# pkusys/Auncel

Hardware: AMD Instinct MI355X
Metric: queries/sec @ recall@10>=0.95, SIFT-10M d=128 IVF4096, 1/2/4/8 GPU (higher is better)
Workload: dtype u8

## Files before the change

### auncel_amd/capi.py

```python
import ctypes as C
import os

import numpy as np

from . import build as _build

METRIC_IP, METRIC_L2 = 0, 1
SUBSET_ID_RANGE, SUBSET_ID_MOD, SUBSET_SLICE, SUBSET_ID_BITS, SUBSET_ID_BATCH = 0, 1, 2, 5, 6
SELECTOR_AND, SELECTOR_OR, SELECTOR_ANDNOT, SELECTOR_NOT = 0, 1, 2, 3

_f32p = C.POINTER(C.c_float)
_i64p = C.POINTER(C.c_int64)
_u64p = C.POINTER(C.c_uint64)
_szp = C.POINTER(C.c_size_t)
_LIB = None

SYMBOLS = [
    "amd_ivf_last_error", "amd_ivf_device_count", "amd_ivf_create", "amd_ivf_clone", "amd_ivf_destroy", "amd_ivf_set_centroids",
    "amd_ivf_set_lists", "amd_ivf_add", "amd_ivf_ntotal", "amd_ivf_list_size", "amd_ivf_get_list", "amd_ivf_coarse",
    "amd_ivf_search_preassigned", "amd_ivf_search", "amd_ivf_scan_codes", "amd_ivf_scan_codes_at", "amd_ivf_scan_codes_range",
    "amd_ivf_scan_codes_range_results", "amd_ivf_distance_to_code", "amd_ivf_stats",
    "amd_ivf_set_queries", "amd_ivf_search_resident", "amd_ivf_search_resident_preassigned", "amd_ivf_coarse_resident", "amd_ivf_set_interdis", "amd_ivf_get_interdis",
    "amd_ivf_set_tuner", "amd_ivf_search_adaptive", "amd_ivf_search_adaptive_x", "amd_ivf_search_adaptive_pre", "amd_ivf_search_timed", "amd_ivf_search_timed_x",
    "amd_ivf_train_samples",
    "amd_ivf_train_samples_x", "amd_ivf_train_samples_pre", "amd_ivf_trace_sb", "amd_ivf_arcos_table", "amd_ivf_merge_tables",
    "amd_ivf_last_timing", "amd_ivf_last_timing_detail", "amd_ivf_last_scan_min_bytes", "amd_ivf_coarse_tie_rows", "amd_ivf_last_tie_fixed", "amd_ivf_last_filter", "amd_ivf_last_direct_out", "amd_ivf_last_coarse_pick", "amd_ivf_set_async_depth", "amd_ivf_submit_adaptive", "amd_ivf_submit_search_resident", "amd_ivf_submit_coarse_resident",
    "amd_ivf_submit_search_resident_preassigned", "amd_ivf_wait", "amd_ivf_async_counts", "amd_ivf_last_tie_redone", "amd_ivf_last_tie_patched", "amd_ivf_self_check", "amd_ivf_last_round_hints", "amd_ivf_set_byte_codes", "amd_ivf_set_option", "amd_ivf_get_option",
    "amd_ivf_kmeans",
    "amd_ivf_range_search_preassigned", "amd_ivf_range_search", "amd_ivf_range_results",
    "amd_ivf_scan_arith",
    "amd_ivf_update_lists", "amd_ivf_remove_ids", "amd_ivf_last_update", "amd_ivf_layout_digest",
    "amd_ivf_subset", "amd_ivf_last_subset",
    "amd_ivf_selector_create", "amd_ivf_selector_destroy", "amd_ivf_selector_info",
    "amd_ivf_search_selected", "amd_ivf_search_preassigned_selected", "amd_ivf_search_resident_selected",
    "amd_ivf_selector_combine", "amd_ivf_range_search_selected", "amd_ivf_range_search_preassigned_selected",
    "amd_ivf_submit_search_resident_selected",
    "amd_ivf_search_selected_each", "amd_ivf_search_preassigned_selected_each", "amd_ivf_search_resident_selected_each",
    "amd_ivf_search_exact", "amd_ivf_search_exact_resident", "amd_ivf_last_exact", "amd_ivf_last_exact_detail",
    "amd_ivf_search_exact_selected", "amd_ivf_search_exact_resident_selected",
    "amd_ivf_range_search_exact", "amd_ivf_range_search_exact_resident", "amd_ivf_range_search_exact_selected", "amd_ivf_last_range_exact",
    "amd_ivf_read_fvecs", "amd_ivf_read_ivecs", "amd_ivf_read_fbin", "amd_ivf_read_ibin", "amd_ivf_free",
]


class EngineError(RuntimeError):
    def __init__(self, code, msg):
        super().__init__(f"auncel_amd error {code}: {msg}")
        self.code = code


def _share_torch_hip_runtime():
    import importlib.util
    import sys
    if "torch" in sys.modules or os.environ.get("AUNCEL_AMD_OWN_HIP_RUNTIME"):
        return
    try:
        spec = importlib.util.find_spec("torch")
    except (ImportError, ValueError):
        return
    if spec is None or not spec.origin:
        return
    d = os.path.join(os.path.dirname(spec.origin), "lib")
    names = ("libhsa-runtime64.so", "libamdhip64.so")
    if not all(os.path.exists(os.path.join(d, n)) for n in names):
        return
    for name in names:
        try:
            _SHARED[name] = C.CDLL(os.path.join(d, name), mode=C.RTLD_GLOBAL)
        except OSError as e:
            raise ImportError(f"auncel_amd: torch's bundled {name} could not be loaded next to {sorted(_SHARED)} ({e}); set "
                              "AUNCEL_AMD_OWN_HIP_RUNTIME=1 to run the engine on ROCm's own runtime (and do not use torch's GPU "
                              "side in the same process)") from e
    if os.environ.get("AUNCEL_AMD_VERBOSE"):
        print(f"[auncel_amd] running on torch's bundled HIP runtime ({d}); AUNCEL_AMD_OWN_HIP_RUNTIME=1 keeps ROCm's", file=sys.stderr)


_SHARED = {}


def hip_runtime():
    import sys
    lib()
    if "libamdhip64.so" in _SHARED:
        return _SHARED["libamdhip64.so"]
    if "torch" in sys.modules:
        p = os.path.join(os.path.dirname(sys.modules["torch"].__file__), "lib", "libamdhip64.so")
        if os.path.exists(p):
            return C.CDLL(p)
    return C.CDLL("libamdhip64.so")


def lib():
    global _LIB
    if _LIB is None:
        if not os.path.exists(_build.LIB):
            raise ImportError(f"{_build.LIB} is missing: run `python -c 'import __graft_entry__ as g; g.build()'` "
                              "(hipcc --offload-arch=gfx950).  auncel_amd has no CPU fallback.")
        _share_torch_hip_runtime()
        L = C.CDLL(os.environ.get("AUNCEL_AMD_LIB", _build.LIB))
        L.amd_ivf_last_error.restype = C.c_char_p
        for s in SYMBOLS[1:]:
            getattr(L, s).restype = C.c_int
        L.amd_ivf_free.restype = None
        _LIB = L
    return _LIB


def _chk(rc):
    if rc != 0:
        raise EngineError(rc, lib().amd_ivf_last_error().decode())
# ... 699 lines not shown
        I = np.empty((n, k), np.int64)
        used = np.zeros(n, np.uint64)
        _chk(lib().amd_ivf_search_timed_x(self._h, C.c_size_t(n), _f(x), C.c_size_t(id_offset), C.c_size_t(k), C.c_size_t(nprobe), _f(b),
                                          coarse_mode, used.ctypes.data_as(_u64p), _f(D), _i(I)))
        return D, I, used

    def train_samples(self, start, n, max_topk, gt_D, train_num, raw, coarse_mode=0):
        gt = f32(gt_D)
        D = np.empty((n, max_topk), np.float32)
        I = np.empty((n, max_topk), np.int64)
        ptrs = (_f32p * len(raw))(*[_f(r) for r in raw])
        _chk(lib().amd_ivf_train_samples(self._h, C.c_size_t(start), C.c_size_t(n), C.c_size_t(max_topk), _f(gt),
                                         C.c_size_t(train_num), coarse_mode, ptrs, _f(D), _i(I)))
        return D, I

    def train_samples_x(self, x, id_offset, max_topk, gt_D, train_num, raw, coarse_mode=0):
        x, gt = f32(x), f32(gt_D)
        n = x.shape[0]
        D = np.empty((n, max_topk), np.float32)
        I = np.empty((n, max_topk), np.int64)
        ptrs = (_f32p * len(raw))(*[_f(r) for r in raw])
        _chk(lib().amd_ivf_train_samples_x(self._h, C.c_size_t(n), _f(x), C.c_size_t(id_offset), C.c_size_t(max_topk), _f(gt),
                                           C.c_size_t(train_num), coarse_mode, ptrs, _f(D), _i(I)))
        return D, I

    def scan_arith(self):
        return int(lib().amd_ivf_scan_arith(self._h))

    def last_timing(self):
        t = (C.c_double * 8)()
        lib().amd_ivf_last_timing(self._h, t)
        mb = C.c_double(0)
        lib().amd_ivf_last_scan_min_bytes(self._h, C.byref(mb))
        return dict(coarse_ms=t[0], scan_ms=t[1], select_ms=t[2], total_ms=t[3], scan_launches=t[4], scan_bytes=t[5],
                    slot_efficiency=t[6], rounds=t[7], scan_min_bytes=mb.value)

    PHASES = ("coarse", "scan_dense", "select_dense", "scan_thr", "select_thr", "tie_fix", "plan")

    def last_timing_detail(self):
        t = (C.c_double * 16)()
        lib().amd_ivf_last_timing_detail(self._h, t)
        d = {p: (t[2 * i], t[2 * i + 1]) for i, p in enumerate(self.PHASES)}
        d["min_bytes_dense"], d["min_bytes_thr"] = t[14], t[15]
        return d

    def coarse_tie_rows(self):
        v = C.c_uint64(0)
        _chk(lib().amd_ivf_coarse_tie_rows(self._h, C.byref(v)))
        return int(v.value)

    def coarse_resident(self, start, n, nprobe, mode=0, want_dis=True):
        keys = np.empty((n, nprobe), np.int64)
        dis = np.empty((n, nprobe), np.float32) if want_dis else None
        _chk(lib().amd_ivf_coarse_resident(self._h, C.c_size_t(start), C.c_size_t(n), C.c_size_t(nprobe), _f(dis), _i(keys), mode))
        return dis, keys

    def search_resident_preassigned(self, start, n, k, keys, out=None):
        keys = i64(keys)
        assert keys.shape[0] == n
        if out is not None:
            D, I = out
        else:
            D = np.empty((n, k), np.float32)
            I = np.empty((n, k), np.int64)
        _chk(lib().amd_ivf_search_resident_preassigned(self._h, C.c_size_t(start), C.c_size_t(n), C.c_size_t(k), C.c_size_t(keys.shape[1]),
                                                       _i(keys), _f(D), _i(I)))
        return D, I

    def last_round_hints(self):
        v = (C.c_uint64 * 2)()
        _chk(lib().amd_ivf_last_round_hints(self._h, v))
        return int(v[0]), int(v[1])

    def last_tie_redone(self):
        v = C.c_uint64(0)
        _chk(lib().amd_ivf_last_tie_redone(self._h, C.byref(v)))
        return int(v.value)

    def last_tie_patched(self):
        v = C.c_uint64(0)
        _chk(lib().amd_ivf_last_tie_patched(self._h, C.byref(v)))
        return int(v.value)

    def last_tie_fixed(self):
        v = C.c_uint64(0)
        _chk(lib().amd_ivf_last_tie_fixed(self._h, C.byref(v)))
        return int(v.value)

    def last_filter(self):
        v = (C.c_uint64 * 2)()
        _chk(lib().amd_ivf_last_filter(self._h, v))
        return int(v[0]), int(v[1])

    def last_direct_out(self):
        return bool(lib().amd_ivf_last_direct_out(self._h))

    def last_coarse_pick(self):
        v = C.c_uint64(0)
        _chk(lib().amd_ivf_last_coarse_pick(self._h, C.byref(v)))
        return int(v.value)

    def set_byte_codes(self, enable):
        lib().amd_ivf_set_byte_codes(self._h, int(bool(enable)))

    def set_option(self, key, value):
        _chk(lib().amd_ivf_set_option(self._h, key.encode(), C.c_double(float("nan") if value is None else float(value))))

    def get_option(self, key):
        v = C.c_double(0)
        _chk(lib().amd_ivf_get_option(self._h, key.encode(), C.byref(v)))
        return v.value
```

### auncel_amd/csrc/ivf_dev.h

```cpp
#pragma once
#include "ivf_kernels.h"

#include <float.h>
#include <utility>

namespace amdivf {

constexpr int64_t REF_TAG = 1ll << 62;

template <bool IsMax> __device__ __forceinline__ bool hcmp(float a, float b) { return IsMax ? a > b : a < b; }
template <bool IsMax> __device__ __forceinline__ float hneutral() { return IsMax ? FLT_MAX : -FLT_MAX; }

template <bool IsMax> __device__ inline void heap_pop(int k, float* val, int64_t* ref) {
    val--;
    ref--;
    const float v = val[k];
    int i = 1;
    for (;;) {
        const int i1 = i << 1, i2 = i1 + 1;
        if (i1 > k) break;
        const int j2 = i2 <= k ? i2 : i1;
        const float c1 = val[i1], c2 = val[j2];
        const int64_t r1 = ref[i1], r2 = ref[j2];
        const bool left = (i2 == k + 1) || hcmp<IsMax>(c1, c2);
        const float c = left ? c1 : c2;
        if (hcmp<IsMax>(v, c)) break;
        val[i] = c;
        ref[i] = left ? r1 : r2;
        i = left ? i1 : i2;
    }
    val[i] = val[k];
    ref[i] = ref[k];
}

template <bool IsMax> __device__ inline void heap_push(int k, float* val, int64_t* ref, float v, int64_t id) {
    val--;
    ref--;
    int i = k;
    while (i > 1) {
        const int f = i >> 1;
        const float fv = val[f];
        if (!hcmp<IsMax>(v, fv)) break;
        val[i] = fv;
        ref[i] = ref[f];
        i = f;
    }
    val[i] = v;
    ref[i] = id;
}

__device__ __forceinline__ uint32_t fkey(float x) {
    const uint32_t u = __float_as_uint(x);
    return u ^ ((uint32_t)((int32_t)u >> 31) | 0x80000000u);
}
__device__ __forceinline__ float fkey_inv(uint32_t key) { return __uint_as_float((key & 0x80000000u) ? key ^ 0x80000000u : ~key); }
template <bool IsMax> __device__ __forceinline__ bool kcmp(uint32_t a, uint32_t b) { return IsMax ? a > b : a < b; }

__device__ __forceinline__ float rl_f(float x, int l) { return __int_as_float(__builtin_amdgcn_readlane(__float_as_int(x), l)); }
__device__ __forceinline__ int rl_i(int x, int l) { return __builtin_amdgcn_readlane(x, l); }
__device__ __forceinline__ uint32_t rl_u(uint32_t x, int l) { return (uint32_t)__builtin_amdgcn_readlane((int)x, l); }

__device__ __forceinline__ uint32_t wave_max_u32(uint32_t x) {
    for (int off = 32; off; off >>= 1) {
        const uint32_t o = (uint32_t)__shfl_xor((int)x, off);
        x = x > o ? x : o;
    }
    return x;
}

__device__ __forceinline__ uint32_t wave_sum_u32(uint32_t x) {
    for (int off = 32; off; off >>= 1) x += (uint32_t)__shfl_xor((int)x, off);
    return x;
}

__device__ __forceinline__ uint32_t wave_err(uint32_t err) { return __ballot(err != 0) ? wave_max_u32(err) : 0u; }

__device__ __forceinline__ void wave_sync() {
    __builtin_amdgcn_fence(__ATOMIC_ACQ_REL, "wavefront");
    __builtin_amdgcn_wave_barrier();
}

template <bool IsMax> __device__ __forceinline__ uint32_t okey(float x) {
    const uint32_t kx = fkey(x);
    return IsMax ? kx : ~kx;
}
template <bool IsMax> __device__ __forceinline__ float okey_inv(uint32_t key) { return fkey_inv(IsMax ? key : ~key); }

struct ItemWalk {
    uint32_t cur, end, step;
    __device__ ItemWalk(uint32_t n, int xcd_chunks) {
        if (xcd_chunks) {
            const uint32_t per = (n + 7) >> 3, x = blockIdx.x & 7;
            cur = x * per + (blockIdx.x >> 3);
            end = (x + 1) * per < n ? (x + 1) * per : n;
            step = gridDim.x >> 3;
        } else {
            cur = blockIdx.x;
            end = n;
            step = gridDim.x;
        }
    }
};


__device__ __forceinline__ uint32_t xcc_id() {
    uint32_t v;
    asm volatile("s_getreg_b32 %0, hwreg(HW_REG_XCC_ID)" : "=s"(v));
    return v & 7u;
}
__device__ __forceinline__ uint32_t xcd_local_add(uint32_t* p, uint32_t v) {
    return __hip_atomic_fetch_add(p, v, __ATOMIC_RELAXED, __HIP_MEMORY_SCOPE_WORKGROUP);
}
__device__ __forceinline__ void xcd_local_add64(unsigned long long* p, unsigned long long v) {
    (void)__hip_atomic_fetch_add(p, v, __ATOMIC_RELAXED, __HIP_MEMORY_SCOPE_WORKGROUP);
}

template <int LANE> __device__ __forceinline__ void writelane_c(int& reg, uint32_t val) {
    asm("v_writelane_b32 %0, %1, %2" : "+v"(reg) : "s"(val), "n"(LANE));
}
template <int METRIC> __device__ __forceinline__ float exact_distance(const float* x, const float* y, int dpad) {
    float s0 = 0.f, s1 = 0.f, s2 = 0.f, s3 = 0.f;
    auto step = [&](const float4& a, const float4& b) {
        if (METRIC == METRIC_L2) {
            const float t0 = b.x - a.x, t1 = b.y - a.y, t2 = b.z - a.z, t3 = b.w - a.w;
            s0 += t0 * t0;
            s1 += t1 * t1;
            s2 += t2 * t2;
            s3 += t3 * t3;
        } else {
            s0 += b.x * a.x;
            s1 += b.y * a.y;
            s2 += b.z * a.z;
            s3 += b.w * a.w;
        }
    };
    int c = 0;
    for (; c + 12 < dpad; c += 16) {
        float4 av[4], bv[4];
#pragma unroll
        for (int u = 0; u < 4; u++) {
            av[u] = *reinterpret_cast<const float4*>(x + c + 4 * u);
            bv[u] = *reinterpret_cast<const float4*>(y + c + 4 * u);
        }
#pragma unroll
        for (int u = 0; u < 4; u++) step(av[u], bv[u]);
    }
    for (; c < dpad; c += 4) step(*reinterpret_cast<const float4*>(x + c), *reinterpret_cast<const float4*>(y + c));
    return (s0 + s1) + (s2 + s3);
}

__device__ __forceinline__ uint32_t list_of_block(const uint64_t* block_off, uint32_t nlist, uint64_t blk) {
    uint32_t lo = 0, hi = nlist;
    while (hi - lo > 1) {
        const uint32_t mid = (lo + hi) >> 1;
        if (block_off[mid] <= blk) lo = mid;
        else hi = mid;
    }
    return lo;
}

template <int... I, class F> __device__ __forceinline__ void static_for(std::integer_sequence<int, I...>, F&& f) {
    (f(std::integral_constant<int, I>{}), ...);
// ... 5 lines not shown
```

### auncel_amd/csrc/ivf_engine.hip

```cpp
#include <hip/hip_runtime.h>

#include <algorithm>
#include <atomic>
#include <cfloat>
#include <cmath>
#include <cstdlib>
#include <chrono>
#include <condition_variable>
#include <deque>
#include <functional>
#include <map>
#include <cstring>
#include <memory>
#include <stdexcept>
#include <string>
#include <mutex>
#include <thread>
#include <unordered_set>
#include <vector>

#include "../../include/auncel_amd.h"
#include "exact_args.h"
#include "ivf_kernels.h"
#include "kmeans_host.h"
// ... 235 lines not shown
    size_t begin(int cat, hipStream_t s) {
        if (off) return NONE;
        Span sp{get(), get(), cat};
        HIP_CHECK(hipEventRecord(sp.a, s));
        spans.push_back(sp);
        return spans.size() - 1;
    }
    void end(size_t i, hipStream_t s) {
        if (i != NONE) HIP_CHECK(hipEventRecord(spans[i].b, s));
    }
    void collect(double* ms_by_cat, int ncat, double* launches_by_cat) {
        for (int c = 0; c < ncat; c++) ms_by_cat[c] = 0, launches_by_cat[c] = 0;
        for (auto& sp : spans) {
            float ms = 0;
            if (hipEventElapsedTime(&ms, sp.a, sp.b) == hipSuccess) {
                ms_by_cat[sp.cat] += ms;
                launches_by_cat[sp.cat] += 1;
            }
            pool.push_back(sp.a);
            pool.push_back(sp.b);
        }
        spans.clear();
    }
    ~EventTimer() {
        for (auto& sp : spans) {
            (void)hipEventDestroy(sp.a);
            (void)hipEventDestroy(sp.b);
        }
        for (auto e : pool) (void)hipEventDestroy(e);
    }
};

enum { CAT_COARSE = 0, CAT_SCAN = 1, CAT_SELECT = 2, CAT_SCAN_THR = 3, CAT_SELECT_THR = 4, CAT_TIE_FIX = 5, CAT_PLAN = 6, NCAT = 7 };

}

struct amd_ivf;
static void async_shutdown(amd_ivf* h);
static bool tickets_out(amd_ivf* h);

struct amd_ivf {
    int d = 0, dpad = 0, metric = METRIC_L2, device = 0;
    size_t nlist = 0, ntotal = 0;
    hipStream_t stream = nullptr;

    std::vector<std::vector<float>> h_codes;
    std::vector<std::vector<int64_t>> h_ids;
    std::vector<uint64_t> h_list_off;
    bool lists_dirty = true;
    bool journal_pending = false;
    std::vector<uint64_t> journal;
    std::vector<IntRange> list_range;
    uint64_t last_update[4] = {0, 0, 0, 0};
    bool is_subset = false;
    uint64_t last_subset[4] = {0, 0, 0, 0};
    PinnedBuf p_upd;
    DevBuf d_upd;
    DevBuf d_codes, d_ids, d_list_off, d_centroids, d_centroid_norms;
    std::vector<float> h_centroids;
    bool have_centroids = false;

    DevBuf d_resident;
    size_t n_resident = 0;
    IntRange db_range, centroid_range, resident_range, call_range;
    int allow_fused = 1;
    int allow_bytes = 1;
    Options opt;
    PinnedBuf p_small;
    size_t small_used = 0;
    struct SmallCopy {
        void* dst;
        size_t off, bytes;
        const void* src;
    };
    std::vector<SmallCopy> small;
    PinnedBuf p_stage;
    size_t stage_used = 0;
    CopySegs h2d_pending{};
    std::vector<std::function<void()>> after_flush;
    bool want_first_tie = false;
    size_t first_tie_nreal = 0;
    DevBuf w_first_tie;
    std::vector<uint32_t> first_tie_host;
    DevBuf w_spec_full, w_spec_dis, w_spec_keys, w_spec_count, w_spec_slot, w_spec_pick, w_redo_idx, w_spec_query, w_spec_scratch, w_split;
    uint32_t spec_cap = 512;
    bool spec_inline = false;
    uint32_t tie_patched_host = 0;
    hipStream_t spec_stream = nullptr;
    hipEvent_t ev_spec_go = nullptr, ev_spec_done = nullptr;
    bool spec_wanted = false;
    bool spec_done = false;
    struct SmallFuse {
        bool active = false, have_init = false, have_bytes = false;
        InitStateArgs init{};
        const float* bx = nullptr;
        int8_t* bout = nullptr;
        int32_t* bcx = nullptr;
    } fuse;
    bool spec_valid = false;
    bool spec_use = false;
    size_t spec_ncopy = 0;
    std::vector<int32_t> spec_slot_host;
    uint64_t tie_rows_host = 0;
    int ties_override = -1;
    int last_arith = 0;
    DevBuf d_frag, d_cy, d_block_off;
    std::vector<uint64_t> h_block_off;
    bool have_codes8 = false;
    DevBuf d_frag32, d_yn;
    std::mutex fp32_gate_mu;
    std::condition_variable fp32_gate_cv;
    int fp32_running = 0;
    uint64_t fp32_gate_next = 0, fp32_gate_serving = 0;
    uint64_t async_served[2] = {0, 0};
    double probed_len = 0;
    DevBuf d_lanes;
    std::atomic<int> lanes_state{0};
    std::atomic<bool> have_frag32{false};
    bool frag32_possible = false;
    DevBuf d_frag16, d_yinfo;
    std::atomic<int> frag16_state{0};
    int allow_filter = 1;
    DevBuf w_xf, w_xn, w_surv, w_surv_cnt;
    DevBuf w_qinfo, w_fparams;

    DevBuf d_interdis;
    bool have_interdis = false;
    DevBuf d_arcos, d_trace_off, d_trace_x, d_trace_y, d_trace_std;
    size_t tuner_max_topk = 0, tuner_ntraces = 0, tuner_trace_cap = 0, tuner_trace_total = 0;
    bool have_tuner = false;

    DevBuf w_qtile, w_group_p0, w_group_cnt, w_xnorms;
    PinnedBuf p_group_p0, p_group_cnt, p_counters;
    DevBuf w_pl_cnt, w_pl_need, w_pl_dist_base, w_pl_lcount, w_pl_lstart, w_pl_gbase, w_pl_ibase, w_pl_fill, w_pl_counters, w_seg_slot;
    DevBuf w_x8, w_xnorm8;
    const float* x8_src = nullptr;
    size_t x8_n = 0;
    uint64_t x8_gen = 0, resident_gen = 1;
    DevBuf w_rcount, w_roff, w_rlab, w_rdis;
    std::vector<size_t> r_lims;
    std::vector<int64_t> r_labels;
    std::vector<uint32_t> r_part_pos;
    std::vector<float> r_part_dis;
    std::vector<float> r_dist;
    DevBuf w_thr, w_mask, w_pl_pad, w_cl_cnt, w_cl_ent, w_cl_arena, w_cl_cursor;
    DevBuf w_x, w_dist, w_items, w_pair_query, w_pair_out, w_seg_off, w_seg_list, w_seg_count, w_qsel;
    DevBuf w_heap_val, w_heap_ref, w_stage, w_nscan, w_done, w_pre_val, w_stoped, w_dtb, w_D, w_I;
    DevBuf w_cdis, w_ckeys, w_stats, w_error, w_misc, w_misc2, w_misc3, w_rawptrs, w_sub_off;
    struct CoarseTail {
        bool valid = false;
        const void* dis = nullptr;
        const void* keys = nullptr;
        size_t prefix = 0, nprobe = 0, rows = 0;
        int metric = 0;
        uint64_t touch_dis = 0, touch_keys = 0;
    } coarse_tail;
    DevBuf c_heap_val, c_heap_ref, c_stage, c_nscan, c_done, c_seg_off, c_seg_list, c_seg_count;
    float centroid_norm_max = 0.f;
    DevBuf d_cinfo;
    bool in_coarse_pick = false;
    size_t coarse_picked = 0;
    DevBuf c_pick_flag, c_pick_x, c_pick_dis, c_pick_keys;
    PinnedBuf p_pick;
    DevBuf c_pair_query, c_pair_out, c_items, c_group_p0, c_group_cnt;
    uint64_t coarse_sig = 0;
    bool coarse_sig_valid = false;
    PinnedBuf p_items, p_pair_query, p_pair_out, p_seg_off, p_seg_list, p_seg_count;
    DevBuf w_seg_begin;
    DevBuf w_log, w_log_cnt, w_amb, w_tie_flag;
    DevBuf w_qstat;
    DevBuf w_keep_each;
    std::vector<uint64_t> keep_each_host;
    DevBuf w_redo_x;
    DevBuf w_log_snap, w_fin_round, w_fix_pos, w_fix_val, w_fix_ref;
    hipStream_t fix_stream = nullptr;
    hipStream_t bg_stream = nullptr;
    hipEvent_t ev_sel = nullptr, ev_fix[2] = {nullptr, nullptr};
    size_t last_state_n = 0;
    DevBuf w_pl_hist;
    PinnedBuf p_hist;
    std::vector<uint32_t> round_hint;
    uint64_t hint_sig = 0;
    uint64_t last_tie_redone = 0;
    uint64_t last_tie_patched = 0;
    uint32_t row_align_now = 1024;
    float* out_D = nullptr;
    int64_t* out_I = nullptr;
    int last_direct_out = 0;
    uint64_t filter_launches = 0;
    uint64_t plan_passes = 0;
    uint64_t hinted_rounds = 0, short_rounds = 0;
    std::atomic<int> live_contexts{1};
    std::atomic<uint64_t> layout_gen{0};
    std::atomic<int> live_selectors{0};
    std::atomic<float> tie_rate{-1.f};
    std::atomic<int> active_searches{0};
    bool force_heap_select = false;
    const int64_t* given_keys = nullptr;
    const float* given_dis = nullptr;
    size_t given_nprobe = 0;
    DevBuf w_ex_blk, w_ex_cnt, w_ex_cand, w_ex_flag, w_ex_tot, w_ex_D, w_ex_I, w_ex_x, w_ex_idx;
    uint64_t last_exact[4] = {0, 0, 0, 0};
    uint64_t last_exact_detail[4] = {0, 0, 0, 0};
    DevBuf w_rx_thr, w_rx_id, w_rx_valid, w_rx_off, w_rx_lab, w_rx_dis;
    uint64_t last_range_exact[4] = {0, 0, 0, 0};
    DevBuf w_limit;
    DevBuf w_tie_rows;

    size_t dist_budget_floats = (size_t)768 << 20;
    WantHistory dist_want;
    std::mutex want_mu;
    WantHistory shared_want;
    size_t stats_host[4] = {0, 0, 0, 0};
    double timing[8] = {0, 0, 0, 0, 0, 0, 0, 0};
    double timing_detail[2 * 7 + 2] = {0};
    double last_min_bytes = 0;
    double scan_bytes = 0, scan_slots = 0, scan_useful = 0, scan_min_bytes = 0, scan_min_bytes_thr = 0;
    EventTimer timer;

    struct AsyncPool* async = nullptr;
    std::vector<amd_ivf*> async_ctx;
    int async_depth = 4;
    amd_ivf* parent = nullptr;
    std::mutex upload_mu;
    std::mutex async_mu;
    hipStream_t aux[4] = {nullptr, nullptr, nullptr, nullptr};
    hipEvent_t ev_fork = nullptr, ev_join[4] = {nullptr, nullptr, nullptr, nullptr};

    ~amd_ivf() {
        async_shutdown(this);
        for (int i = 0; i < 4; i++) {
            if (aux[i]) (void)hipStreamDestroy(aux[i]);
            if (ev_join[i]) (void)hipEventDestroy(ev_join[i]);
        }
        if (ev_fork) (void)hipEventDestroy(ev_fork);
        if (bg_stream) (void)hipStreamDestroy(bg_stream);
        if (ev_spec_go) (void)hipEventDestroy(ev_spec_go);
        if (ev_spec_done) (void)hipEventDestroy(ev_spec_done);
        if (ev_sel) (void)hipEventDestroy(ev_sel);
        for (int i = 0; i < 2; i++)
            if (ev_fix[i]) (void)hipEventDestroy(ev_fix[i]);
        if (stream) (void)hipStreamDestroy(stream);
    }
};

static inline amd_ivf* ix(amd_ivf* h) { return h->parent ? h->parent : h; }
static inline const amd_ivf* ix(const amd_ivf* h) { return h->parent ? h->parent : h; }
static inline double opt(const amd_ivf* h, OptId id, double dflt) { return ix(h)->opt.get(id, dflt); }

namespace {

void use_device(const amd_ivf* h) { HIP_CHECK(hipSetDevice(h->device)); }

hipError_t stream_sync(hipStream_t s) {
    static const bool blocking = [] {
        const char* e = getenv("AUNCEL_AMD_BLOCKING_SYNC");
        return e && *e && *e != '0';
    }();
    if (!blocking) return hipStreamSynchronize(s);
    thread_local hipEvent_t ev = nullptr;
    thread_local int ev_dev = -1;
    int dev = 0;
    hipError_t e = hipGetDevice(&dev);
    if (e != hipSuccess) return e;
    if (!ev || ev_dev != dev) {
        e = hipEventCreateWithFlags(&ev, hipEventBlockingSync | hipEventDisableTiming);
// ... 1914 lines not shown
    auto fetch_counters = [&](size_t nhist, bool with_stats = false) {
        if (pinned_io(h)) {
            CopySegs c{};
            c.src[0] = h->w_pl_counters.p;
            c.dst[0] = h->p_counters.dev();
            c.words[0] = (uint32_t)CNT_WORDS;
            c.n = 1;
            if (nhist) {
                c.src[c.n] = h->w_pl_hist.p;
                c.dst[c.n] = h->p_hist.dev();
                c.words[c.n] = (uint32_t)(nhist * 16);
                c.n++;
            }
            if (with_stats) {
                c.src[c.n] = h->w_stats.p;
                c.dst[c.n] = static_cast<unsigned char*>(h->p_counters.dev()) + CNT_WORDS * 4;
                c.words[c.n] = (uint32_t)STAT_WORDS;
                c.n++;
            }
            launch_copy_segs(c, s);
        } else {
            HIP_CHECK(hipMemcpyAsync(hc, h->w_pl_counters.p, CNT_WORDS * 4, hipMemcpyDeviceToHost, s));
            if (nhist) HIP_CHECK(hipMemcpyAsync(h->p_hist.p, h->w_pl_hist.p, nhist * 64, hipMemcpyDeviceToHost, s));
        }
    };
    auto plan_and_look = [&](size_t round_len) {
        plan_round(round_len);
        fetch_counters(0);
        HIP_CHECK(stream_sync(s));
    };
    auto epilogue = [h, hc, chained, hints_used, bsig](size_t nh) {
        if (chained) {
            h->round_hint.assign(h->p_hist.as<uint32_t>(), h->p_hist.as<uint32_t>() + nh * 16);
            h->round_hint.insert(h->round_hint.end(), hc, hc + 16);
            static const bool dbg_rounds = getenv("AUNCEL_AMD_DEBUG_ROUNDS") != nullptr;
            if (dbg_rounds)
                for (size_t r = 0; (r + 1) * 16 <= h->round_hint.size(); r++) {
                    const uint32_t* c = &h->round_hint[r * 16];
                    fprintf(stderr, "[rounds] %zu: queries %u segments %u pairs %u groups %u items qg1 %u qg2 %u qg4 %u qg8 %u\n", r, c[CNT_ACTIVE],
                            c[CNT_SEGMENTS], c[CNT_PAIRS], c[CNT_GROUPS], c[CNT_QG1], c[CNT_QG2], c[CNT_QG4], c[CNT_QG8]);
                }
            for (size_t r = 0; (r + 1) * 16 <= hints_used.size() && (r + 1) * 16 <= h->round_hint.size(); r++)
                for (int c : {CNT_QG1, CNT_QG2, CNT_QG4, CNT_QG8}) {
                    const uint32_t used = hints_used[r * 16 + c], need = h->round_hint[r * 16 + c];
                    if (!used) continue;
                    h->hinted_rounds++;
                    if (need > used + used / 8 + 8) h->short_rounds++;
                }
        }
        if (chained) {
            uint32_t want_mi = hc[12];
            for (size_t r = 0; r < nh; r++) want_mi = std::max(want_mi, h->p_hist.as<uint32_t>()[r * 16 + 12]);
            size_t want = (size_t)want_mi << 20;
            h->dist_want.raise(bsig, want);
            amd_ivf* owner = ix(h);
            std::lock_guard<std::mutex> lock(owner->want_mu);
            owner->shared_want.raise(bsig, want);
        }
        h->scan_bytes += *reinterpret_cast<double*>(hc + 16);
        h->scan_min_bytes += *reinterpret_cast<double*>(hc + 22);
        h->scan_min_bytes_thr += *reinterpret_cast<double*>(hc + 24 + PLAN_MAX_ROUNDS * 8);
        const unsigned long long* acc = reinterpret_cast<const unsigned long long*>(hc + 18);
        h->scan_slots += (double)acc[0];
        h->scan_useful += (double)acc[1];
    };
    static const bool no_skip = getenv("AUNCEL_AMD_NO_LAST_PLAN_SKIP") != nullptr;
    size_t round_len = first_round;

    if (chained) {
        const size_t padded = (maxlist + 1023) & ~(size_t)1023;
        const bool fits = (double)n * (double)total_nprobe * (double)padded <= (double)budget && n * total_nprobe <= round_pairs;
        bool fixed_complete = !base.tuner.enabled && !base.train.enabled && fits && (base.fixed_two || first_round >= total_nprobe);
        static const size_t ahead_env = getenv("AUNCEL_AMD_ROUNDS_AHEAD") ? (size_t)atoi(getenv("AUNCEL_AMD_ROUNDS_AHEAD")) : 0;
        size_t batch = ahead_env ? ahead_env : base.train.enabled ? 4 : base.tuner.enabled ? (n < 20 ? 1 : 2) : (base.fixed_two ? 2 : 1);
        if (fixed_complete) batch = base.fixed_two && first_round < total_nprobe ? 2 : 1;
        bool planned = false;
        for (size_t round = 0;;) {
            for (size_t b = 0; b < batch; b++, round++) {
                const bool thr_mode = round > 0 && !no_thr;
                if (!planned) plan_round(round_len);
                planned = false;
                launch_due_fix();
                enqueue_scan(thr_mode, nullptr, round);
                if (round == 0 && base.split_prepare && !thr_mode && active.before == 0) {
                    base.split_prepare();
                    enqueue_replay(thr_mode, (uint32_t)n, true, round, base.split_free, base.split_counts);
                    base.split_between();
                    enqueue_replay(thr_mode, base.split_wait_cap, true, round, base.split_wait, base.split_counts + 1);
                } else {
                    if (round == 0 && base.before_first_select) base.before_first_select();
                    enqueue_replay(thr_mode, (uint32_t)n, true, round);
                }
                round_len = next_round_len(round_len);
            }
            launch_due_fix();
            if (fixed_complete) break;
            static const bool plan_look = getenv("AUNCEL_AMD_PLAN_LOOK") != nullptr;
            if (!plan_look && round >= 1 && round - 1 < PLAN_MAX_ROUNDS) {
                const bool speculate = base.spec_finish && pinned_io(h) && round == 1 && planned_rounds == 1 && !fix_pending && !eager_fix;
                const size_t small_mark = h->small.size(), af_mark = h->after_flush.size(), used_mark = h->small_used;
                fetch_counters(0, speculate);
                if (speculate) {
                    base.spec_finish();
                    launch_small_gathers(h, s);
                }
                host_stamp("enqueued");
                HIP_CHECK(stream_sync(s));
                host_stamp("look-sync");
                uint32_t unf = 0;
                for (int x = 0; x < 8; x++) unf += hc[24 + (round - 1) * 8 + x];
                const uint32_t left = unf + hc[11];
                if (speculate) {
                    const unsigned long long* rows = reinterpret_cast<const unsigned long long*>(hc + CNT_WORDS);
                    unsigned long long flagged = 0;
                    for (uint32_t r = 0; r < STATS_ROWS; r++) flagged += rows[4 * r + 3];
                    if (left == 0 && flagged == 0) {
                        flush_small(h);
                        std::vector<std::function<void()>> fs;
                        fs.swap(h->after_flush);
                        h->spec_done = true;
                        for (auto& f : fs) f();
                        epilogue(0);
                        return;
                    }
                    h->small.resize(small_mark);
                    h->after_flush.resize(af_mark);
                    h->small_used = used_mark;
                }
                if (dbg_timing()) fprintf(stderr, "[rounds/chained] after round %zu: unfinished %u deferred %u\n", round, unf, hc[11]);
                if (left == 0) break;
                plan_round(round_len);
            } else {
                plan_and_look(round_len);
                if (dbg_timing())
                    fprintf(stderr, "[rounds/chained] after round %zu: active %u pairs %u items %u may-continue %u MiB %u\n", round, hc[CNT_ACTIVE],
                            hc[CNT_PAIRS], hc[CNT_QG1] + hc[CNT_QG2] + hc[CNT_QG4] + hc[CNT_QG8], hc[10], hc[7]);
                if (hc[CNT_ACTIVE] == 0) break;
            }
            planned = true;
            batch = ahead_env ? ahead_env : 2;
        }
    } else {
        for (size_t round = 0;; round++) {
            const bool thr_mode = base.range || (round > 0 && !no_thr);
            const double t0 = now_us();
            if (base.d_budget_ms) {
                HIP_CHECK(stream_sync(s));
                pa.elapsed_ms = (float)((now_us() - base.t_start_us) * 1e-3);
            }
            plan_and_look(round_len);
            const double t1 = now_us();
            const uint32_t nact = hc[CNT_ACTIVE];
            if (nact == 0) break;
            enqueue_scan(thr_mode, hc, round);
            if (base.range) {
                RangeArgs ga{};
                ga.nq = nact;
                ga.nlist = (uint32_t)nlist;
                ga.qsel = h->w_qsel.as<uint32_t>();
                ga.seg_count = h->w_pl_cnt.as<uint32_t>();
                ga.seg_begin = h->w_seg_begin.as<uint32_t>();
                ga.seg_list = h->w_seg_list.as<int32_t>();
                ga.seg_off = h->w_seg_off.as<uint64_t>();
                ga.list_off = I->d_list_off.as<uint64_t>();
                ga.ids = I->d_ids.as<int64_t>();
                ga.dist = h->w_dist.as<float>();
                ga.mask = h->w_mask.as<unsigned long long>();
// ... 896 lines not shown
        h->w_ckeys.ensure(n * nlist * 8);
        HIP_CHECK(hipStreamWaitEvent(h->stream, h->ev_spec_done, 0));
        launch_spec_gather(h->w_spec_pick.as<int32_t>(), (uint32_t)n, (uint32_t)nlist, (uint32_t)h->spec_ncopy, h->w_spec_dis.as<float>(),
                           h->w_spec_keys.as<int64_t>(), h->w_cdis.as<float>(), h->w_ckeys.as<int64_t>(), h->stream);
        h->tie_rows_host += n;
        return nlist;
    }
    if (!h->given_keys) {
        h->w_cdis.ensure(n * nlist * 4);
        h->w_ckeys.ensure(n * nlist * 8);
        coarse_dev(h, d_x, n, nlist, coarse_mode, h->w_cdis.as<float>(), h->w_ckeys.as<int64_t>(), fused_ok, coarse_prefix);
        return nlist;
    }
    const size_t np = h->given_nprobe;
    if (np <= nlist / 8 + 20) throw EngineError("tune / train mode reads coarse entries 0 .. nlist/8 + 20: nprobe too small");
    h->w_cdis.ensure(n * np * 4);
    h->w_ckeys.ensure(n * np * 8);
    HIP_CHECK(hipMemcpyAsync(h->w_cdis.p, h->given_dis, n * np * 4, hipMemcpyHostToDevice, h->stream));
    HIP_CHECK(hipMemcpyAsync(h->w_ckeys.p, h->given_keys, n * np * 8, hipMemcpyHostToDevice, h->stream));
    return np;
}

static size_t coarse_read_bound(size_t nlist, float multipler, const uint64_t* my_nprobe, size_t n) {
    size_t bound = std::max<size_t>(nlist / 8 + 21, (size_t)((double)(nlist / 8) * (double)multipler) + 2);
    for (size_t i = 0; i < n; i++) bound = std::max<size_t>(bound, (size_t)my_nprobe[i] + 1);
    return bound + 16;
}

static void adaptive_core_once(amd_ivf_t* h, const float* d_x, size_t start, size_t n, size_t query_topk, float multipler, float std_m,
                            const float* require_acc, const float* gt_D, int profile, int coarse_mode,
                            uint64_t* my_nprobe, float* t_recalls, float* D, int64_t* I, const IntRange& qr) {
    use_device(h);
    CallScope call_scope(h);
    const amd_ivf* owner = ix(h);
    if (!owner->have_tuner || !owner->have_interdis)
        throw EngineError("Search tune start can't start without IVF_pro init and training");
    if (n == 0) return;
    const size_t K = owner->tuner_max_topk, nlist = h->nlist;
    if (nlist <= nlist / 8 + 20) throw EngineError("tune mode needs nprobe(=nlist) > nlist/8 + 20");
    size_t ntr = 0;
    while (((size_t)1 << ntr) <= nlist / 8) ntr++;
    if (owner->tuner_ntraces < ntr) throw EngineError("not enough traces for this nlist");
    if (query_topk == 0 || query_topk > K) throw EngineError("query_topk out of range");
    {
        const int pt = (int)opt(h, OPT_PHASE_TIMING, -1);
        h->timer.off = pt >= 0 ? pt == 0 : n < 20;
    }
    g_stamps.clear();
    host_stamp("begin");
    WallClock wc(h->stream, h->timer.off);
    upload_lists(h);
    host_stamp("clock+lists");
    const size_t nabs = start + n;
    DevBuf &d_req = h->w_misc2, &d_np = h->w_misc3;
    const size_t ncap = std::max(nabs, resident_owner(h)->n_resident);
    d_req.ensure(ncap * 4 * 2 + (gt_D ? ncap * K * 4 : 0) + 64);
    float* dreq = d_req.as<float>();
    float* dtr = dreq + ncap;
    float* dgt = gt_D ? dtr + ncap : nullptr;
    d_np.ensure(ncap * 8);
    h2d_small(h, dreq + start, require_acc + start, n * 4, h->stream);
    h2d_small(h, dtr + start, t_recalls + start, n * 4, h->stream);
    if (gt_D) HIP_CHECK(hipMemcpyAsync(dgt + start * K, gt_D + start * K, n * K * 4, hipMemcpyHostToDevice, h->stream));
    h2d_small(h, d_np.as<unsigned long long>() + start, my_nprobe + start, n * 8, h->stream);
    flush_h2d(h, h->stream);
    host_stamp("inputs");

    size_t coarse_prefix = coarse_read_bound(nlist, multipler, my_nprobe + start, n);
    if (coarse_prefix >= nlist || getenv("AUNCEL_AMD_FULL_COARSE_SORT")) coarse_prefix = 0;

    reset_scan_counters(h);
    unsigned long long* const dnp = d_np.as<unsigned long long>();
    const auto tail_gathers = [&]() {
        d2h_small(h, my_nprobe + start, dnp + start, n * 8, h->stream);
        d2h_small(h, t_recalls + start, dtr + start, n * 4, h->stream);
        if (h->want_first_tie) {
            h->first_tie_host.assign(n, 0);
            d2h_small(h, h->first_tie_host.data(), h->w_first_tie.p, n * 4, h->stream);
            if (h->spec_valid) {
                h->spec_slot_host.assign(n, -1);
                d2h_small(h, h->spec_slot_host.data(), h->w_spec_slot.p, n * 4, h->stream);
                h->tie_patched_host = 0;
                if (h->spec_inline) d2h_small(h, &h->tie_patched_host, h->w_spec_count.as<uint32_t>() + 1, 4, h->stream);
            }
        }
    };
    h->spec_done = false;
    SmallCopies pending(h);

    const size_t np_row = coarse_or_given(h, d_x, n, coarse_mode, ix(h)->allow_fused && ix(h)->centroid_range.fusable_with(qr, h->metric), coarse_prefix);
    host_stamp("coarse");
    const bool fuse_small = n <= 4 && !h->spec_wanted;
    if (h->want_first_tie) {
        h->w_first_tie.ensure(n * 4);
        static const bool no_spec = getenv("AUNCEL_AMD_NO_TIE_SPECULATION") != nullptr;
        const uint32_t SPEC_CAP = n <= 5120 ? 512u : (uint32_t)(((n / 8 + 63) / 64) * 64);
        constexpr uint32_t SPEC_NEAR = 64, SPEC_WINDOW = 2 * (12 + 144) + 14;
        h->spec_cap = SPEC_CAP;
        h->spec_valid = false;
        const bool can_spec = !no_spec && h->spec_wanted && !h->given_keys && np_row == nlist && n <= h->dist_budget_floats / std::max<size_t>(nlist, 1) &&
                              heap_tie_order_lds((uint32_t)nlist, (uint32_t)nlist) <= 160 * 1024;
        if (!can_spec && !fuse_small)
            launch_first_tie(h->w_cdis.as<float>(), (uint32_t)n, (uint32_t)nlist, (uint32_t)h->first_tie_nreal, h->w_first_tie.as<uint32_t>(), h->stream);
        if (can_spec) {
            const size_t ncopy = std::min(h->first_tie_nreal, nlist);
            h->w_spec_full.ensure((size_t)SPEC_CAP * nlist * 4);
            h->w_spec_dis.ensure((size_t)SPEC_CAP * nlist * 4);
            h->w_spec_keys.ensure((size_t)SPEC_CAP * nlist * 8);
            h->w_spec_count.ensure(32);
            h->w_spec_slot.ensure(n * 4);
            h->w_spec_query.ensure((size_t)SPEC_CAP * 4);
            ensure_context_streams(h);
            HIP_CHECK(hipStreamWaitEvent(h->stream, h->ev_spec_done, 0));
            HIP_CHECK(hipMemsetAsync(h->w_spec_count.p, 0, 32, h->stream));
            (void)SPEC_NEAR;
            launch_tie_collect(h->w_cdis.as<float>(), (uint32_t)n, (uint32_t)h->first_tie_nreal, SPEC_WINDOW, SPEC_CAP, (uint32_t)nlist, (uint32_t)ncopy,
                               h->w_dist.as<float>(), h->w_ckeys.as<int64_t>(), h->w_first_tie.as<uint32_t>(), h->w_spec_count.as<uint32_t>(),
                               h->w_spec_slot.as<int32_t>(), h->w_spec_full.as<float>(), h->w_spec_dis.as<float>(), h->w_spec_keys.as<int64_t>(),
                               h->w_spec_query.as<uint32_t>(), h->stream);
            HIP_CHECK(hipEventRecord(h->ev_spec_go, h->stream));
            HIP_CHECK(hipStreamWaitEvent(h->spec_stream, h->ev_spec_go, 0));
            launch_heap_tie_order(h->w_spec_full.as<float>(), SPEC_CAP, (uint32_t)nlist, (uint32_t)nlist, (uint32_t)ncopy, h->metric,
                                  h->w_spec_dis.as<float>(), h->w_spec_keys.as<int64_t>(),
                                  reinterpret_cast<unsigned long long*>(h->w_spec_count.as<uint32_t>() + 2), h->spec_stream,
                                  h->w_spec_count.as<uint32_t>());
            HIP_CHECK(hipEventRecord(h->ev_spec_done, h->spec_stream));
            h->spec_valid = true;
            h->spec_ncopy = ncopy;
            static const bool no_patch = getenv("AUNCEL_AMD_NO_TIE_PATCH") != nullptr;
            h->spec_inline = !no_patch && (nlist & (nlist - 1)) == 0 && nlist >= 64;
        }
    }
    const bool tie_inline = h->want_first_tie && h->spec_valid && h->spec_inline;
    struct FuseScope {
        amd_ivf* h;
        bool on;
        FuseScope(amd_ivf* hh, bool o) : h(hh), on(o) {
            if (on) {
                h->fuse = amd_ivf::SmallFuse{};
                h->fuse.active = true;
            }
        }
        ~FuseScope() { h->fuse.active = false; }
    } fuse_scope(h, fuse_small);
    init_state(h, n, K, true);
    auto set_online = [h, nlist, n, np_row](const uint32_t* only = nullptr, const uint32_t* only_count = nullptr, uint32_t cap = 0) {
        launch_set_online(h->metric, (uint32_t)nlist, only ? cap : (uint32_t)n, h->w_cdis.as<float>(), h->w_ckeys.as<int64_t>(), (uint32_t)np_row,
                          ix(h)->d_interdis.as<float>(), ix(h)->d_arcos.as<float>(), h->w_dtb.as<float>(), h->w_error.as<uint32_t>(), h->stream,
                          only, only_count);
    };
    if (!fuse_small && !tie_inline) set_online();
    RoundSpec base;
    if (tie_inline) {
        size_t maxlist = 0;
        for (size_t l = 0; l < nlist; l++) maxlist = std::max<size_t>(maxlist, ix(h)->h_list_off[l + 1] - ix(h)->h_list_off[l]);
        const size_t SCRATCH_FLOATS = std::min<size_t>((size_t)64 << 20, std::max<size_t>((size_t)8 << 20, (size_t)h->spec_cap * 16 * ((maxlist + 1023) & ~(size_t)1023)));
        h->w_spec_scratch.ensure(SCRATCH_FLOATS * 4);
        base.run_ties = true;
        base.before_first_select = [h, nlist, set_online, SCRATCH_FLOATS]() {
            HIP_CHECK(hipStreamWaitEvent(h->stream, h->ev_spec_done, 0));
            TiePatchArgs ta{};
            ta.count = h->w_spec_count.as<uint32_t>();
            ta.cap = h->spec_cap;
            ta.nlist = (uint32_t)nlist;
            ta.ncopy = (uint32_t)h->spec_ncopy;
            ta.key_stride = (uint32_t)nlist;
            ta.slot_query = h->w_spec_query.as<uint32_t>();
            ta.slot_of = h->w_spec_slot.as<int32_t>();
            ta.s_keys = h->w_spec_keys.as<int64_t>();
            ta.ckeys = h->w_ckeys.as<int64_t>();
            ta.seg_count = h->w_pl_cnt.as<uint32_t>();
            ta.seg_begin = h->w_seg_begin.as<uint32_t>();
            ta.seg_list = h->w_seg_list.as<int32_t>();
            ta.seg_off = h->w_seg_off.as<uint64_t>();
            ta.list_off = ix(h)->d_list_off.as<uint64_t>();
            ta.dist = h->w_dist.as<float>();
            ta.row_align = h->row_align_now;
            ta.scratch = h->w_spec_scratch.as<float>();
            ta.scratch_floats = SCRATCH_FLOATS;
            ta.cursor = reinterpret_cast<unsigned long long*>(h->w_spec_count.as<uint32_t>() + 4);
            ta.patched = h->w_spec_count.as<uint32_t>() + 1;
            launch_tie_patch(ta, h->stream);
            set_online();
        };
        static const bool no_split = getenv("AUNCEL_AMD_NO_SPLIT_SELECT") != nullptr;
        if (!no_split && n >= 256) {
            h->w_split.ensure((2 * n + 8) * 4);
            uint32_t* counts = h->w_split.as<uint32_t>();
            uint32_t* q_free = counts + 8;
            uint32_t* q_wait = q_free + n;
            const auto patch_hook = base.before_first_select;
            const uint32_t wait_cap = (uint32_t)std::min<size_t>(n, h->spec_cap);
            base.split_free = q_free;
            base.split_wait = q_wait;
            base.split_counts = counts;
            base.split_wait_cap = wait_cap;
            base.split_prepare = [h, n, counts, q_free, q_wait, set_online]() {
                HIP_CHECK(hipMemsetAsync(counts, 0, 8, h->stream));
                launch_partition_qsel(nullptr, nullptr, (uint32_t)n, h->w_spec_slot.as<int32_t>(), q_free, q_wait, counts, h->stream);
                set_online();
            };
            base.split_between = [h, patch_hook, counts, q_wait, wait_cap, set_online]() {
                (void)set_online;
                patch_hook();
            };
        }
    }
    base.fused = ix(h)->allow_fused && ix(h)->db_range.fusable_with(qr, h->metric);
    base.bytes = byte_queries(h, ix(h), d_x, n, qr);
    if (fuse_small) {
        h->fuse.active = false;
        SmallStateArgs sa{};
        sa.init = h->fuse.init;
        sa.metric = h->metric;
        sa.nlist = (uint32_t)nlist;
        sa.nq = (uint32_t)n;
        sa.coarse_dis = h->w_cdis.as<float>();
        sa.coarse_keys = h->w_ckeys.as<int64_t>();
        sa.coarse_stride = (uint32_t)np_row;
        sa.interdis = ix(h)->d_interdis.as<float>();
        sa.arcos = ix(h)->d_arcos.as<float>();
        sa.dtb = h->w_dtb.as<float>();
        if (h->want_first_tie) {
            sa.ft_sorted_dis = h->w_cdis.as<float>();
            sa.ft_stride = (uint32_t)nlist;
            sa.ft_nreal = (uint32_t)h->first_tie_nreal;
            sa.ft_out = h->w_first_tie.as<uint32_t>();
        }
        if (h->fuse.have_bytes) {
            sa.bx = h->fuse.bx;
            sa.bout = h->fuse.bout;
            sa.bcx = h->fuse.bcx;
        }
        sa.d = h->d;
        sa.dpad = h->dpad;
        launch_small_state(sa, h->stream);
    }
    ix(h)->last_arith = base.bytes ? 2 : base.fused ? 1 : 0;
    base.k = (int)K;
    base.id_offset = start;
    base.d_x = d_x;
    base.d_cdis = h->w_cdis.as<float>();
    base.d_ckeys = h->w_ckeys.as<int64_t>();
    base.coarse_stride = (uint32_t)np_row;
    base.tuner = make_tuner(h, query_topk, multipler, std_m, dreq, dgt, dnp, dtr, profile);
    const size_t first_env = std::max<size_t>(1, (size_t)opt(h, OPT_ROUND_FIRST, 12));
    base.caller_checks_error = true;
    DirectOut direct(h, D, I);
    host_stamp("state");
    if (n < 20)
        base.spec_finish = [&]() {
            finish_results(h, n, K, D, I, nullptr, true);
            tail_gathers();
        };
    run_rounds_device(h, base, n, first_env, np_row, dnp);
    host_stamp("rounds");
    if (!h->spec_done) {
        finish_results(h, n, K, D, I, nullptr, true);
        tail_gathers();
        sync_and_flush(h, h->stream);
    }
    h->spec_done = false;
    host_stamp("final-sync");
    const double wall = wc.stop();
    host_stamp("clock");
    print_stamps();
    double ms[NCAT], ln[NCAT];
    h->timer.collect(ms, NCAT, ln);
    fill_timing(h, ms, ln);
    h->timer.off = false;
    h->timing[3] = wall;
    h->timing[5] = h->scan_bytes;
    h->last_min_bytes = h->scan_min_bytes;
    h->timing[6] = h->scan_slots > 0 ? h->scan_useful / h->scan_slots : 0;
}

static void adaptive_redo_ties(amd_ivf_t* h, const float* d_x, size_t start, size_t n, size_t query_topk, float multipler, float std_m,
                               const float* require_acc, const float* gt_D, int profile, int coarse_mode, uint64_t* my_nprobe,
                               float* t_recalls, float* D, int64_t* I, const IntRange& qr) {
    const size_t K = ix(h)->tuner_max_topk, nlist = h->nlist;
    const std::vector<uint64_t> np0(my_nprobe + start, my_nprobe + start + n);
    const std::vector<float> tr0(t_recalls + start, t_recalls + start + n);
    const size_t nreal = std::min(coarse_read_bound(nlist, multipler, np0.data(), n), nlist);
    TieRegime regime(h);
    h->ties_override = 0;
    h->want_first_tie = true;
    h->first_tie_nreal = nreal;
    h->spec_valid = false;
    h->spec_wanted = true;
    with_select_fallback(h, [&] { adaptive_core_once(h, d_x, start, n, query_topk, multipler, std_m, require_acc, gt_D, profile, coarse_mode, my_nprobe, t_recalls, D, I, qr); });
    h->want_first_tie = false;
    h->spec_wanted = false;
    std::vector<uint32_t> again;
    const bool patched = h->spec_inline && h->spec_valid && h->spec_slot_host.size() == n;
    for (size_t i = 0; i < n; i++) {
        const uint64_t bound = 2 * my_nprobe[start + i] + 14;
        const bool in_order = patched && h->spec_slot_host[i] >= 0 && bound <= h->spec_ncopy;
        if ((h->first_tie_host[i] < bound && !in_order) || bound + 1 >= nreal) again.push_back((uint32_t)i);
    }
    h->last_tie_redone = again.size();
    h->last_tie_patched = patched ? h->tie_patched_host : 0;
    if (again.empty()) return;
    const size_t m = again.size();
    std::vector<unsigned long long> nscan(n);
    std::vector<uint2> qstat(n);
    HIP_CHECK(hipMemcpyAsync(nscan.data(), h->w_nscan.p, n * 8, hipMemcpyDeviceToHost, h->stream));
    HIP_CHECK(hipMemcpyAsync(qstat.data(), h->w_qstat.p, n * sizeof(uint2), hipMemcpyDeviceToHost, h->stream));
    bool spec = h->spec_valid && h->spec_slot_host.size() == n;
    std::vector<int32_t> pick(m, -1);
    for (size_t j = 0; j < m && spec; j++) {
        pick[j] = h->spec_slot_host[again[j]];
        if (pick[j] <= -2) pick[j] = -2 - pick[j];
        spec = pick[j] >= 0;
    }
    if (getenv("AUNCEL_AMD_DEBUG_REDO")) {
        size_t have = 0, nslots = 0;
        for (size_t j = 0; j < m; j++) have += h->spec_valid && h->spec_slot_host.size() == n && h->spec_slot_host[again[j]] >= 0;
        for (int32_t v : h->spec_slot_host) nslots += v >= 0;
        fprintf(stderr, "[redo] n %zu again %zu spec_valid %d slots given %zu, of the queries searched again %zu have one -> %s\n", n, m,
                (int)h->spec_valid, nslots, have, spec ? "slots" : "heap in the second pass");
    }
    h->w_redo_x.ensure(m * h->dpad * sizeof(float));
    h->w_redo_idx.ensure(m * 4);
    HIP_CHECK(hipMemcpyAsync(h->w_redo_idx.p, again.data(), m * 4, hipMemcpyHostToDevice, h->stream));
    launch_gather_rows(d_x, h->w_redo_idx.as<uint32_t>(), (uint32_t)m, (uint32_t)h->dpad, h->w_redo_x.as<float>(), h->stream);
    if (spec) {
        h->w_spec_pick.ensure(m * 4);
        HIP_CHECK(hipMemcpyAsync(h->w_spec_pick.p, pick.data(), m * 4, hipMemcpyHostToDevice, h->stream));
    }
    HIP_CHECK(stream_sync(h->stream));
    for (size_t j = 0; j < m; j++) {
        h->stats_host[0] -= 1;
        h->stats_host[1] -= qstat[again[j]].x;
        h->stats_host[2] -= nscan[again[j]];
        h->stats_host[3] -= qstat[again[j]].y;
    }
    std::vector<float> req(m), tr(m), Dc(m * K), gt;
    std::vector<uint64_t> np(m);
    std::vector<int64_t> Ic(m * K);
    if (gt_D) gt.resize(m * K);
    for (size_t j = 0; j < m; j++) {
        const size_t id = start + again[j];
        req[j] = require_acc[id];
        np[j] = np0[again[j]];
        tr[j] = tr0[again[j]];
        if (gt_D) std::copy(gt_D + id * K, gt_D + (id + 1) * K, gt.begin() + j * K);
    }
    h->ties_override = 1;
    h->spec_use = spec;
    with_select_fallback(h, [&] {
        adaptive_core_once(h, h->w_redo_x.as<float>(), 0, m, query_topk, multipler, std_m, req.data(), gt_D ? gt.data() : nullptr, profile,
                           coarse_mode, np.data(), tr.data(), Dc.data(), Ic.data(), qr);
    });
    for (size_t j = 0; j < m; j++) {
        const size_t i = again[j];
        my_nprobe[start + i] = np[j];
        t_recalls[start + i] = tr[j];
        std::copy(Dc.begin() + j * K, Dc.begin() + (j + 1) * K, D + i * K);
        std::copy(Ic.begin() + j * K, Ic.begin() + (j + 1) * K, I + i * K);
    }
}

static void adaptive_core(amd_ivf_t* h, const float* d_x, size_t start, size_t n, size_t query_topk, float multipler, float std_m,
                          const float* require_acc, const float* gt_D, int profile, int coarse_mode,
                          uint64_t* my_nprobe, float* t_recalls, float* D, int64_t* I, const IntRange& qr) {
    const int ties_opt = (int)opt(h, OPT_COARSE_TIES, -1);
    const bool can_speculate = !h->given_keys && n > 0 && h->nlist > 128 && multipler >= 1.f && !(profile & 2);
    const bool speculate = can_speculate && n < 20 && ties_opt < 0;
    const bool redo_some = can_speculate && n >= 20 && ties_opt == 2;
    if (redo_some) {
        adaptive_redo_ties(h, d_x, start, n, query_topk, multipler, std_m, require_acc, gt_D, profile, coarse_mode, my_nprobe, t_recalls, D, I, qr);
        return;
    }
    if (!speculate) {
        with_select_fallback(h, [&] { adaptive_core_once(h, d_x, start, n, query_topk, multipler, std_m, require_acc, gt_D, profile, coarse_mode, my_nprobe, t_recalls, D, I, qr); });
        return;
    }
    size_t stats0[4];
    for (int i = 0; i < 4; i++) stats0[i] = h->stats_host[i];
    const std::vector<uint64_t> np0(my_nprobe + start, my_nprobe + start + n);
    const std::vector<float> tr0(t_recalls + start, t_recalls + start + n);
    const size_t nreal = std::min(coarse_read_bound(h->nlist, multipler, np0.data(), n), h->nlist);
    TieRegime regime(h);
    h->ties_override = 0;
// ... 358 lines not shown
                            idx_out.as<uint32_t>(), counts.as<uint32_t>(), temp.p, temp_bytes, s);
        HIP_CHECK(hipMemcpyAsync(cnt.data(), counts.p, (k + 1) * 4, hipMemcpyDeviceToHost, s));
        HIP_CHECK(stream_sync(s));
        if (cnt[k]) throw EngineError("k-means: the assignment step returned a centroid number outside [0, k)");
        float err = 0;
        for (size_t j = 0; j < nx; j++) err += dis[j];
        if (obj) obj[it] = err;
        off[0] = 0;
        for (size_t c = 0; c < k; c++) {
            off[c + 1] = off[c] + cnt[c];
            hassign[c] = cnt[c];
        }
        HIP_CHECK(hipMemcpyAsync(seg.p, off.data(), (k + 1) * 4, hipMemcpyHostToDevice, s));
        launch_kmeans_sums(h->d_resident.as<float>(), dpad, d, idx_out.as<uint32_t>(), seg.as<uint32_t>(), (uint32_t)k, d_cen.as<float>(), s);
        HIP_CHECK(hipMemcpyAsync(centroids, d_cen.p, k * (size_t)d * 4, hipMemcpyDeviceToHost, s));
        HIP_CHECK(stream_sync(s));
        km::split_void_clusters(centroids, hassign, d, k, nx);
        km::post_process(centroids, d, k, spherical != 0, int_centroids != 0);
    }
    API_END
}

int amd_ivf_scan_arith(amd_ivf_t* h) { return ix(h)->last_arith; }

int amd_ivf_set_byte_codes(amd_ivf_t* h, int enable) {
    h->allow_bytes = enable ? 1 : 0;
    for (amd_ivf* c : h->async_ctx) c->allow_bytes = h->allow_bytes;
    return 0;
}

static int opt_id(const char* key) {
    if (key)
        for (int i = 0; i < N_OPT; i++)
            if (!strcmp(key, OPT_TABLE[i].key)) return i;
    throw EngineError(std::string("unknown option: ") + (key ? key : "(null)"));
}
static double opt_default(OptId id) {
    switch (id) {
        case OPT_COARSE_TIES: case OPT_TIE_FIX: case OPT_PHASE_TIMING: return -1;
        case OPT_FIXED_ROUNDS: case OPT_ROUND_INC: case OPT_ROUND_GROW: case OPT_EXACT_FLOAT: case OPT_EXACT_WIDE: case OPT_EXACT_WIDE_BYTES: return 0;
        case OPT_ROUND_FIRST: return 12;
        case OPT_SCAN_PIPELINED: return 7;
        case OPT_FILTER: case OPT_COARSE_PICK: return 2;
        case OPT_ROW_LISTS: return ROW_LISTS_DEFAULT;
        case OPT_EXACT_SEED_NPROBE: return EXACT_SEED_DEFAULT;
        default: return 1;
    }
}
int amd_ivf_set_option(amd_ivf_t* h, const char* key, double value) {
    API_BEGIN
    if (!h) throw EngineError("null handle");
    ix(h)->opt.v[opt_id(key)].store(std::isnan(value) ? OPT_UNSET : value, std::memory_order_relaxed);
    API_END
}
int amd_ivf_get_option(amd_ivf_t* h, const char* key, double* value) {
    API_BEGIN
    if (!h || !value) throw EngineError("null argument");
    const OptId id = (OptId)opt_id(key);
    *value = opt(h, id, opt_default(id));
    API_END
}

int amd_ivf_last_scan_min_bytes(amd_ivf_t* h, double* bytes) {
    *bytes = h->last_min_bytes;
    return 0;
}

int amd_ivf_last_round_hints(amd_ivf_t* h, uint64_t out[2]) {
    out[0] = h->hinted_rounds;
    out[1] = h->short_rounds;
    return 0;
}

int amd_ivf_last_tie_redone(amd_ivf_t* h, uint64_t* queries) {
    *queries = h->last_tie_redone;
    return 0;
}

int amd_ivf_last_tie_patched(amd_ivf_t* h, uint64_t* rankings) {
    *rankings = h->last_tie_patched;
    return 0;
}

int amd_ivf_last_tie_fixed(amd_ivf_t* h, uint64_t* queries) {
    API_BEGIN
    use_device(h);
    *queries = 0;
    if (h->w_tie_flag.p && h->last_state_n) {
        std::vector<uint32_t> f(h->last_state_n);
        HIP_CHECK(stream_sync(h->stream));
        HIP_CHECK(hipMemcpy(f.data(), h->w_tie_flag.p, f.size() * 4, hipMemcpyDeviceToHost));
        for (uint32_t v : f) *queries += v == 2;
    }
    API_END
}
int amd_ivf_last_direct_out(amd_ivf_t* h) { return h ? h->last_direct_out : 0; }
int amd_ivf_last_coarse_pick(amd_ivf_t* h, uint64_t* rankings) {
    *rankings = h ? h->coarse_picked : 0;
    return 0;
}
int amd_ivf_last_filter(amd_ivf_t* h, uint64_t out[2]) {
    API_BEGIN
    use_device(h);
    out[0] = h->filter_launches;
    out[1] = 0;
    if (h->filter_launches && h->w_surv_cnt.p) {
        uint32_t v = 0;
        HIP_CHECK(stream_sync(h->stream));
        HIP_CHECK(hipMemcpy(&v, h->w_surv_cnt.p, 4, hipMemcpyDeviceToHost));
        out[1] = v;
    }
    API_END
}
int amd_ivf_coarse_tie_rows(amd_ivf_t* h, uint64_t* rows) {
    API_BEGIN
    use_device(h);
    *rows = h->tie_rows_host;
    if (h->w_tie_rows.p) {
        uint64_t v = 0;
        HIP_CHECK(stream_sync(h->stream));
        HIP_CHECK(hipMemcpy(&v, h->w_tie_rows.p, 8, hipMemcpyDeviceToHost));
        *rows += v;
    }
    API_END
}

int amd_ivf_last_timing(amd_ivf_t* h, double out[8]);
int amd_ivf_last_scan_min_bytes(amd_ivf_t* h, double* bytes);
int amd_ivf_last_round_hints(amd_ivf_t* h, uint64_t out[2]);
int amd_ivf_last_tie_redone(amd_ivf_t* h, uint64_t* queries);
int amd_ivf_last_direct_out(amd_ivf_t* h);

}

struct amd_ivf_selector {
    amd_ivf* index = nullptr;
    uint64_t gen = 0;
    DevBuf keep;
    DevBuf count;
    DevBuf list_kept;
    uint64_t info[4] = {0, 0, 0, 0};
    mutable int tickets = 0;
};

struct AdaptiveSpec {
    size_t start = 0, n = 0, query_topk = 0;
    float multipler = 0.f, std_m = 0.f;
    const float* require_acc = nullptr;
    const float* gt_D = nullptr;
    int profile = 0, coarse_mode = 0;
    uint64_t* my_nprobe = nullptr;
    float* t_recalls = nullptr;
    float* D = nullptr;
    int64_t* I = nullptr;
};
struct AsyncJob {
    std::function<int(amd_ivf_t*)> run;
    bool adaptive = false;
    AdaptiveSpec spec;
    const amd_ivf_selector* sel = nullptr;
    uint32_t coalesced = 1;
    int rc = 0;
    bool done = false;
    std::string error;
    double timing[9] = {0, 0, 0, 0, 0, 0, 0, 0, 0};
    uint64_t diag[4] = {0, 0, 0, 0};
// ... 1585 lines not shown
```

### auncel_amd/csrc/ivf_kernels.h

```cpp
#pragma once
#include <hip/hip_runtime.h>
#include <stddef.h>
#include <stdint.h>
#include <stdio.h>
#include <stdlib.h>
#include <string.h>

#include <stdexcept>
#include <string>

#include "selector_args.h"

namespace amdivf {

inline void check_launch(const char* what) {
    const hipError_t e = hipGetLastError();
    if (e != hipSuccess) throw std::runtime_error(std::string("kernel launch failed: ") + what + ": " + hipGetErrorString(e));
    static const bool sync_each = getenv("AUNCEL_AMD_SYNC_LAUNCH") != nullptr;
    if (sync_each) {
        fprintf(stderr, "[launch] %.100s\n", what);
        const hipError_t s = hipDeviceSynchronize();
        if (s != hipSuccess) throw std::runtime_error(std::string("kernel failed: ") + what + ": " + hipGetErrorString(s));
    }
}
// ... 235 lines not shown
    uint32_t* log_snap;
    uint32_t nq_total;
    uint32_t* fin_round;
    uint2* qstat;
    uint32_t* unfinished;
    const uint32_t* cl_cnt;
    const uint2* cl_ent;
    const uint2* cl_arena;
};

bool replay_sorted_applies(const ReplayArgs& a);
void launch_replay(const ReplayArgs& a, hipStream_t s);

constexpr uint32_t CL_CAP = 8;
constexpr uint32_t CL_WALK = 0xffffffffu;
struct CompactArgs {
    const uint32_t* nseg_dev;
    uint32_t nseg;
    uint32_t nseg_hint;
    uint32_t nlist;
    const int32_t* seg_list;
    const uint64_t* seg_off;
    const uint64_t* list_off;
    const float* dist;
    const unsigned long long* mask;
    uint32_t* cl_cnt;
    uint2* cl_ent;
    uint2* arena;
    uint32_t arena_per_xcd;
    uint32_t* cursor;
};
void launch_compact_rows(const CompactArgs& a, hipStream_t s);

struct TieFixArgs {
    int metric;
    int k;
    uint32_t nq, nlist;
    const uint2* log;
    uint32_t log_cap;
    uint32_t round;
    int final_pass;
    const uint32_t* log_cnt;
    const uint32_t* log_snap;
    const uint32_t* fin_round;
    float* fix_val;
    int64_t* fix_ref;
    uint32_t* fix_pos;
    uint32_t* tie_flag;
    const uint64_t* list_off;
    const int64_t* ids;
    int store_pairs, identity_ids;
    float* D;
    int64_t* I;
};
void launch_tie_fix(const TieFixArgs& a, hipStream_t s);

struct RangeArgs {
    uint32_t nq;
    uint32_t nlist;
    const uint32_t* qsel;
    const uint32_t* seg_count;
    const uint32_t* seg_begin;
    const int32_t* seg_list;
    const uint64_t* seg_off;
    const uint64_t* list_off;
    const int64_t* ids;
    const float* dist;
    const unsigned long long* mask;
    uint32_t* counts;
    const unsigned long long* out_off;
    int64_t* out_labels;
    float* out_dist;
    uint32_t* stage;
    uint32_t* done;
    unsigned long long* stats;
    uint32_t* error;
};
void launch_range_count(const RangeArgs& a, hipStream_t s);
void launch_range_fill(const RangeArgs& a, hipStream_t s);

void launch_set_online(int metric, uint32_t nlist, uint32_t nq, const float* coarse_dis, const int64_t* coarse_keys,
                       uint32_t coarse_stride, const float* interdis, const float* arcos, float* dtb, uint32_t* error, hipStream_t s,
                       const uint32_t* qsel = nullptr, const uint32_t* nq_dev = nullptr);
void launch_partition_qsel(const uint32_t* qsel, const uint32_t* nq_dev, uint32_t nq, const int32_t* slot_of, uint32_t* q_free, uint32_t* q_wait,
                           uint32_t* counts, hipStream_t s);

struct PlanArgs {
    uint32_t nq;
    uint32_t nlist;
    uint32_t total_nprobe;
    uint32_t key_stride;
    uint32_t slot_base;
    uint32_t first_round, round_len;
    uint32_t min_inc;
    int tune;
    int d;
    float multipler;
    double grow;
    unsigned long long id_offset;
    unsigned long long dist_budget;
    uint32_t seg_cap;
    const int64_t* keys;
    const uint64_t* list_off;
    const uint32_t* stage;
    const uint32_t* done;
    const unsigned long long* my_nprobe;
    const float* budget_ms;
    float elapsed_ms;
    uint32_t* limit;
    uint32_t* cnt;
    unsigned long long* need;
    uint32_t* pad;
    uint32_t row_align;
    uint32_t qblock;
    uint32_t mfma_chunk;
    uint32_t mfma_qblock;
    int item_order;
    const uint64_t* block_off;
    const uint64_t* lane_block_off;
    uint32_t* seg_begin;
    unsigned long long* dist_base;
    uint32_t* qsel;
    int32_t* seg_list;
    uint64_t* seg_off;
    uint32_t* lcount;
    uint32_t* lstart;
    uint32_t* gbase;
    uint32_t* ibase;
    uint32_t* xcount;
    uint32_t* seg_slot;
    uint32_t* pair_query;
    uint64_t* pair_out;
    uint32_t* group_p0;
    uint32_t* group_cnt;
    ScanItem* items;
    uint32_t item_cap;
    uint32_t* error;
    unsigned long long* acc64;
    uint32_t* history;
    int first_plan;
    uint32_t* round_unfinished;
    uint32_t* cl_cursor;
    uint32_t* counters;
    double* bytes;
    double* min_bytes;
    double* min_bytes_thr;
    uint32_t row_bytes;
    int dense_round;
    const float* run_dis;
};

void launch_xcd_check(uint32_t* counters, uint32_t nkeys, uint32_t* slot, uint32_t* xcc_of, uint32_t n, hipStream_t s);

constexpr uint32_t PLAN_MAX_ROUNDS = 64;
constexpr uint32_t STATS_ROWS = 9;
void launch_plan(const PlanArgs& a, hipStream_t s);

constexpr uint32_t ERR_ARCOS_DOMAIN = 1;
constexpr uint32_t ERR_COSINE_PRECOND = 2;
constexpr uint32_t ERR_INVALID_KEY = 3;
constexpr uint32_t ERR_ITEM_OVERFLOW = 4;
constexpr uint32_t ERR_LOG_OVERFLOW = 5;

bool sort_rows_ranks_a_prefix(uint32_t nlist, uint32_t nprobe, uint32_t prefix);
void launch_sort_rows(const float* dis, uint32_t nq, uint32_t nlist, uint32_t nprobe, int metric, float* out_dis,
                      int64_t* out_keys, hipStream_t s, uint32_t prefix = 0, bool tail_is_neutral = false);

bool launch_heap_tie_order(const float* dis, uint32_t nq, uint32_t nlist, uint32_t nprobe, uint32_t nout, int metric, float* out_dis,
                           int64_t* out_keys, unsigned long long* nrows, hipStream_t s, const uint32_t* dev_nq = nullptr);

size_t heap_tie_order_lds(uint32_t nlist, uint32_t nprobe);

void launch_spec_collect(const uint32_t* first, uint32_t nq, uint32_t lo, uint32_t window, uint32_t cap, uint32_t nlist, uint32_t ncopy,
                         const float* full, const float* cdis, const int64_t* ckeys, uint32_t* count, int32_t* slot_of, float* s_full,
                         float* s_dis, int64_t* s_keys, hipStream_t s, uint32_t* slot_query = nullptr);
struct TiePatchArgs {
    const uint32_t* count;
    uint32_t cap, nlist, ncopy, key_stride;
    const uint32_t* slot_query;
    int32_t* slot_of;
    const int64_t* s_keys;
    int64_t* ckeys;
    const uint32_t* seg_count;
    const uint32_t* seg_begin;
    int32_t* seg_list;
    uint64_t* seg_off;
    const uint64_t* list_off;
    float* dist;
    uint32_t row_align;
    float* scratch;
    unsigned long long scratch_floats;
    unsigned long long* cursor;
    uint32_t* patched;
};
void launch_tie_patch(const TiePatchArgs& a, hipStream_t s);
void launch_tie_collect(const float* sorted_dis, uint32_t nq, uint32_t nreal, uint32_t window, uint32_t cap, uint32_t nlist, uint32_t ncopy,
                        const float* full, const int64_t* ckeys, uint32_t* first_out, uint32_t* count, int32_t* slot_of, float* s_full, float* s_dis,
                        int64_t* s_keys, uint32_t* slot_query, hipStream_t s);
void launch_spec_gather(const int32_t* slots, uint32_t m, uint32_t nlist, uint32_t ncopy, const float* s_dis, const int64_t* s_keys,
                        float* cdis, int64_t* ckeys, hipStream_t s);
void launch_gather_rows(const float* x, const uint32_t* idx, uint32_t m, uint32_t dpad, float* out, hipStream_t s);

void launch_first_tie(const float* sorted_dis, uint32_t nq, uint32_t stride, uint32_t nreal, uint32_t* out, hipStream_t s);

void launch_row_norms(const float* x, size_t n, int d, float* out, hipStream_t s);
void launch_coarse_gemm16(int metric, const float* X, const float* Y, const float* xn, const float* yn, int nq, int ny, int d, float* out,
                          const FilterParams* params, hipStream_t s);
void launch_coarse_gemm(int metric, const float* X, const float* Y, const float* xn, const float* yn, int nq, int ny, int d, float* out,
                        hipStream_t s);

void launch_coarse_pick(int metric, const float* approx, const float* x, const float* centroids, const float* xn, float cmax, uint32_t n,
                        uint32_t nlist, uint32_t nprobe, int dpad, float* out_dis, int64_t* out_keys, uint32_t* nflag, uint32_t* flagged,
                        hipStream_t s, const FilterParams* params = nullptr, uint32_t* why = nullptr);
void launch_scatter_rows(const void* in, const uint32_t* idx, uint32_t m, uint32_t words, void* out, hipStream_t s);

void launch_pack_upper(const float* full, uint32_t nlist, float* out, hipStream_t s);

size_t kmeans_sort_temp_bytes(size_t n);
void launch_kmeans_group(const int64_t* assign, size_t n, uint32_t k, uint32_t* keys_in, uint32_t* keys_out, uint32_t* idx_in,
                         uint32_t* idx_out, uint32_t* counts, void* temp, size_t temp_bytes, hipStream_t s);
void launch_kmeans_sums(const float* x, size_t stride, int d, const uint32_t* idx_sorted, const uint32_t* seg_off, uint32_t k, float* centroids,
                        hipStream_t s);

struct CopySegs {
    static constexpr int MAX = 12;
    const void* src[MAX];
    void* dst[MAX];
    uint32_t words[MAX];
    uint32_t n;
};
void launch_copy_segs(const CopySegs& c, hipStream_t s);

struct InitStateArgs {
    size_t n, k;
    float neutral;
    float* heap_val;
    int64_t* heap_ref;
    float* thr;
    uint32_t* stage;
    unsigned long long* nscan;
    uint32_t* done;
    float* pre_val;
    uint32_t* stoped;
    unsigned long long* stats;
    uint32_t* error;
    uint32_t *log_cnt, *amb, *tie_flag;
    uint32_t *log_snap, *fin_round, *fix_pos;
    uint2* qstat;
    float* fix_val;
    int64_t* fix_ref;
};
void launch_init_state(const InitStateArgs& a, hipStream_t s);
struct SmallStateArgs {
    InitStateArgs init;
    int metric;
    uint32_t nlist, nq;
    const float* coarse_dis;
    const int64_t* coarse_keys;
    uint32_t coarse_stride;
    const float* interdis;
    const float* arcos;
    float* dtb;
    const float* ft_sorted_dis;
    uint32_t ft_stride, ft_nreal;
    uint32_t* ft_out;
    const float* bx;
    int d, dpad;
    int8_t* bout;
    int32_t* bcx;
};
void launch_small_state(const SmallStateArgs& a, hipStream_t s);
void launch_range_collect(const float* dist, uint32_t n, float radius, int metric, uint32_t* count, uint32_t* out_pos, float* out_dis, hipStream_t s);
void launch_fill_f32(float* p, size_t n, float v, hipStream_t s);
void launch_fill_i64(int64_t* p, size_t n, int64_t v, hipStream_t s);

void launch_frag_from_f32_list(const float* codes, const uint64_t* list_off, const uint64_t* block_off, uint32_t nlist, const uint64_t* blocks,
                               uint64_t nlisted, int d, int dpad, int metric, uint8_t* out, int32_t* cy, hipStream_t s);
void launch_frag32_from_f32_list(const float* codes, const uint64_t* list_off, const uint64_t* block_off, uint32_t nlist, const uint64_t* blocks,
                                 uint64_t nlisted, int d, int dpad, int metric, float* out, float* yn, hipStream_t s);
void launch_frag16_from_f32_list(const float* codes, const uint64_t* list_off, const uint64_t* block_off, uint32_t nlist, const uint64_t* blocks,
                                 uint64_t nlisted, int d, int dpad, int metric, const uint32_t* info, float* out, float* yn, hipStream_t s);
// ... 164 lines not shown
```

### auncel_amd/csrc/ivf_kernels.hip

```cpp
#include "ivf_dev.h"

#include <float.h>
#include <algorithm>
#include <stdexcept>
#include <stdlib.h>
#include <string>
#include <type_traits>
#include <utility>

namespace amdivf {

#ifndef AUNCEL_SCAN_PF
#define AUNCEL_SCAN_PF 2
#endif
typedef float f2 __attribute__((ext_vector_type(2)));
constexpr int LDS_ROW = SCAN_DC + 4;

template <int QG> struct ScanShape {
    static constexpr int NT = QG == 8 ? 512 : QG == 1 ? 64 : 256;
    static constexpr int vg = QG >= 4 || QG == 1 ? 1 : 4 / QG;
    static constexpr int tile_vecs = vg * SCAN_WAVE_VECS;
    static constexpr int lds_floats = tile_vecs * LDS_ROW;
};

// ... 2056 lines not shown
#endif
    __builtin_amdgcn_s_setprio(AUNCEL_HEAP_WAVE_PRIO);
    HeapEnt* h = reinterpret_cast<HeapEnt*>(smem);
    const bool fast = nprobe == nlist && (nlist & (nlist - 1)) == 0 && nlist >= 64;
    float* row = fast ? nullptr : reinterpret_cast<float*>(smem + (size_t)(nprobe + 2) * 8);
    const uint32_t q = blockIdx.x, lane = threadIdx.x;
    const float* grow = dis + (size_t)q * nlist;
    float* od = out_dis + (size_t)q * nprobe;
    int64_t* ok = out_keys + (size_t)q * nprobe;
    const float neutral = IsMax ? FLT_MAX : -FLT_MAX;
    const uint32_t nreal = nout < nlist ? nout : nlist;
    bool tie = false;
    for (uint32_t i = lane; i + 1 < nreal; i += 64) tie |= od[i] == od[i + 1];
    if (nreal && nreal < nlist) {
        const float T = od[nreal - 1];
        uint32_t in_row = 0, in_out = 0;
        for (uint32_t j = lane; j < nlist; j += 64) in_row += grow[j] == T;
        for (uint32_t i = lane; i < nreal; i += 64) in_out += od[i] == T;
        in_row = wave_sum_u32(in_row);
        in_out = wave_sum_u32(in_out);
        tie |= in_row > in_out;
    }
    if (!__ballot(tie)) return;
    bool enters = true;
    for (uint32_t j = lane; j < nlist; j += 64) {
        const float v = grow[j];
        if (row) row[j] = v;
        enters &= hcmp<IsMax>(neutral, v);
    }
    for (uint32_t i = lane; i < nprobe + 2; i += 64) h[i] = HeapEnt{neutral, 0xffffffffu};
    wave_sync();
    if (lane == 0) atomicAdd(nrows, 1ull);
    if (fast && !__ballot(!enters)) {
        floyd_fill_pow2<IsMax>(h, grow, nlist, (int)lane);
        heapsort_pipelined<IsMax>(h, nlist, ok, nout < nprobe ? nout : nprobe, (int)lane);
        return;
    }
    if (!row) {
        row = const_cast<float*>(grow);
    }
    uint32_t nvalid = 0;
    if (lane == 0) {
        const uint32_t k = nprobe;
        for (uint32_t j = 0; j < nlist; j++) {
            const float dj = row[j];
            if (hcmp<IsMax>(h[1].v, dj)) {
                lds_heap_pop<IsMax>(h, k);
                lds_heap_push<IsMax>(h, k, dj, j);
            }
        }
        uint32_t ii = 0;
        for (uint32_t i = 0; i < k; i++) {
            const HeapEnt top = h[1];
            lds_heap_pop<IsMax>(h, k - i);
            h[k - ii] = top;
            if (top.id != 0xffffffffu) ii++;
        }
        nvalid = ii;
    }
    wave_sync();
    nvalid = (uint32_t)__builtin_amdgcn_readfirstlane((int)nvalid);
    for (uint32_t i = lane; i < nout && i < nprobe; i += 64) {
        const bool real = i < nvalid;
        const HeapEnt e = real ? h[nprobe - nvalid + 1 + i] : HeapEnt{neutral, 0xffffffffu};
        od[i] = e.v;
        ok[i] = real ? (int64_t)e.id : -1;
    }
}

__global__ __launch_bounds__(64) void first_tie_kernel(const float* sorted_dis, uint32_t stride, uint32_t nreal, uint32_t* out) {
    const float* od = sorted_dis + (size_t)blockIdx.x * stride;
    uint32_t first = 0xffffffffu;
    for (uint32_t i = threadIdx.x; i + 1 < nreal; i += 64)
        if (od[i] == od[i + 1] && i < first) first = i;
    for (int off = 32; off; off >>= 1) {
        const uint32_t o = (uint32_t)__shfl_xor((int)first, off);
        first = o < first ? o : first;
    }
    if (threadIdx.x == 0) out[blockIdx.x] = first;
}

__global__ __launch_bounds__(64) void tie_collect_kernel(const float* sorted_dis, uint32_t nreal, uint32_t window, uint32_t cap, uint32_t nlist,
                                                         uint32_t ncopy, const float* full, const int64_t* ckeys, uint32_t* first_out, uint32_t* count,
                                                         int32_t* slot_of, float* s_full, float* s_dis, int64_t* s_keys, uint32_t* slot_query) {
    const uint32_t q = blockIdx.x, lane = threadIdx.x;
    const float* od = sorted_dis + (size_t)q * nlist;
    uint32_t first = 0xffffffffu;
    for (uint32_t i = lane; i + 1 < nreal; i += 64)
        if (od[i] == od[i + 1] && i < first) first = i;
    for (int off = 32; off; off >>= 1) {
        const uint32_t o = (uint32_t)__shfl_xor((int)first, off);
        first = o < first ? o : first;
    }
    if (lane == 0) first_out[q] = first;
    uint32_t slot = 0xffffffffu;
    if (lane == 0 && first < window) slot = atomicAdd(count, 1u);
    slot = (uint32_t)__builtin_amdgcn_readfirstlane((int)slot);
    if (slot >= cap) {
        if (lane == 0) slot_of[q] = -1;
        return;
    }
    if (lane == 0) {
        slot_of[q] = (int32_t)slot;
        slot_query[slot] = q;
    }
    const float* fr = full + (size_t)q * nlist;
    float* fo = s_full + (size_t)slot * nlist;
    for (uint32_t j = lane; j < nlist; j += 64) fo[j] = fr[j];
    for (uint32_t j = lane; j < ncopy; j += 64) {
        s_dis[(size_t)slot * nlist + j] = od[j];
        s_keys[(size_t)slot * nlist + j] = ckeys[(size_t)q * nlist + j];
    }
}

void launch_tie_collect(const float* sorted_dis, uint32_t nq, uint32_t nreal, uint32_t window, uint32_t cap, uint32_t nlist, uint32_t ncopy,
                        const float* full, const int64_t* ckeys, uint32_t* first_out, uint32_t* count, int32_t* slot_of, float* s_full, float* s_dis,
                        int64_t* s_keys, uint32_t* slot_query, hipStream_t s) {
    if (nq)
        LAUNCH(tie_collect_kernel, dim3(nq), dim3(64), 0, s, sorted_dis, nreal, window, cap, nlist, ncopy, full, ckeys, first_out, count, slot_of, s_full,
               s_dis, s_keys, slot_query);
}

void launch_first_tie(const float* sorted_dis, uint32_t nq, uint32_t stride, uint32_t nreal, uint32_t* out, hipStream_t s) {
    if (nq) LAUNCH(first_tie_kernel, dim3(nq), dim3(64), 0, s, sorted_dis, stride, nreal, out);
}

__global__ __launch_bounds__(64) void spec_collect_kernel(const uint32_t* first, uint32_t lo, uint32_t window, uint32_t cap, uint32_t nlist, uint32_t ncopy,
                                                          const float* full, const float* cdis, const int64_t* ckeys, uint32_t* count,
                                                          int32_t* slot_of, float* s_full, float* s_dis, int64_t* s_keys, uint32_t* slot_query) {
    const uint32_t q = blockIdx.x, lane = threadIdx.x;
    uint32_t slot = 0xffffffffu;
    if (first[q] < lo) return;
    if (lane == 0 && first[q] < window) slot = atomicAdd(count, 1u);
    slot = (uint32_t)__builtin_amdgcn_readfirstlane((int)slot);
    if (slot >= cap) {
        if (lane == 0) slot_of[q] = -1;
        return;
    }
    if (lane == 0) {
        slot_of[q] = (int32_t)slot;
        if (slot_query) slot_query[slot] = q;
    }
    const float* fr = full + (size_t)q * nlist;
    float* fo = s_full + (size_t)slot * nlist;
    for (uint32_t j = lane; j < nlist; j += 64) fo[j] = fr[j];
    for (uint32_t j = lane; j < ncopy; j += 64) {
        s_dis[(size_t)slot * nlist + j] = cdis[(size_t)q * nlist + j];
        s_keys[(size_t)slot * nlist + j] = ckeys[(size_t)q * nlist + j];
    }
}

void launch_spec_collect(const uint32_t* first, uint32_t nq, uint32_t lo, uint32_t window, uint32_t cap, uint32_t nlist, uint32_t ncopy,
                         const float* full, const float* cdis, const int64_t* ckeys, uint32_t* count, int32_t* slot_of, float* s_full,
                         float* s_dis, int64_t* s_keys, hipStream_t s, uint32_t* slot_query) {
    if (nq)
        LAUNCH(spec_collect_kernel, dim3(nq), dim3(64), 0, s, first, lo, window, cap, nlist, ncopy, full, cdis, ckeys, count, slot_of, s_full, s_dis, s_keys,
               slot_query);
}

__global__ __launch_bounds__(64) void tie_patch_kernel(TiePatchArgs a) {
    const uint32_t slot = blockIdx.x, lane = threadIdx.x;
    const uint32_t nslots = *a.count < a.cap ? *a.count : a.cap;
    if (slot >= nslots) return;
    const uint32_t q = a.slot_query[slot];
    const int64_t* nk = a.s_keys + (size_t)slot * a.nlist;
    int64_t* ok = a.ckeys + (size_t)q * a.key_stride;
    const uint32_t cnt0 = a.seg_count[q];
    bool changed = false, in_round = false;
    for (uint32_t j = lane; j < a.ncopy; j += 64) {
        const int64_t want = nk[j];
        if (ok[j] != want) {
            ok[j] = want;
            changed = true;
            in_round = in_round || j < cnt0;
        }
    }
    if (!__ballot(changed)) return;
    if (lane == 0) atomicAdd(a.patched, 1u);
    if (!__ballot(in_round)) return;
    auto give_up = [&]() {
        if (lane == 0) a.slot_of[q] = -2 - (int32_t)slot;
    };
    if (cnt0 > 64) return give_up();
    const uint32_t seg0 = a.seg_begin[q];
    const bool in = lane < cnt0;
    const int32_t oldkey = in ? a.seg_list[seg0 + lane] : -1;
    const int32_t newkey = in ? (int32_t)nk[lane] : -1;
    const unsigned long long off_old = in ? a.seg_off[seg0 + lane] : 0ull;
    unsigned long long psz = 0;
    if (in && oldkey >= 0 && (uint32_t)oldkey < a.nlist) {
        const unsigned long long sz = a.list_off[oldkey + 1] - a.list_off[oldkey], ra = a.row_align - 1;
        psz = (sz + ra) & ~ra;
    }
    int src = -1;
    for (uint32_t p = 0; p < cnt0; p++)
        if (rl_i(oldkey, (int)p) == newkey) src = (int)p;
    if (__ballot(in && (src < 0 || newkey < 0)) != 0) return give_up();
    const unsigned long long moved = __ballot(in && src != (int)lane);
    if (!moved) return;
    const int lo = __builtin_ctzll(moved), hi = 63 - __builtin_clzll(moved);
    const uint32_t my_psz = (uint32_t)psz;
    uint32_t new_psz = (uint32_t)__shfl((int)my_psz, src < 0 ? 0 : src);
    const bool span = (int)lane >= lo && (int)lane <= hi;
    uint32_t incl = span ? new_psz : 0u;
    for (int off = 1; off < 64; off <<= 1) {
        const uint32_t o = (uint32_t)__shfl_up((int)incl, off);
        if ((int)lane >= off) incl += o;
    }
    const uint32_t total = (uint32_t)__shfl((int)incl, hi);
    const unsigned long long base = ((unsigned long long)rl_u((uint32_t)(off_old >> 32), lo) << 32) | rl_u((uint32_t)off_old, lo);
    const unsigned long long off_new = base + (incl - (span ? new_psz : 0u));
    unsigned long long at = 0;
    if (lane == 0) at = atomicAdd(a.cursor, (unsigned long long)total);
    at = ((unsigned long long)(uint32_t)__builtin_amdgcn_readfirstlane((int)(at >> 32)) << 32) | (uint32_t)__builtin_amdgcn_readfirstlane((int)(uint32_t)at);
    if (at + total > a.scratch_floats) return give_up();
    float* sc = a.scratch + at;
    for (uint32_t i = lane; i < total; i += 64) sc[i] = a.dist[base + i];
    __threadfence();
    wave_sync();
    for (int p = lo; p <= hi; p++) {
        const int sp = rl_i(src, p);
        const unsigned long long from = (((unsigned long long)rl_u((uint32_t)(off_old >> 32), sp) << 32) | rl_u((uint32_t)off_old, sp)) - base;
        const unsigned long long to = ((unsigned long long)rl_u((uint32_t)(off_new >> 32), p) << 32) | rl_u((uint32_t)off_new, p);
        const uint32_t len = rl_u(new_psz, p);
        for (uint32_t i = lane; i < len; i += 64) a.dist[to + i] = sc[from + i];
    }
    if (span) {
        a.seg_list[seg0 + lane] = newkey;
        a.seg_off[seg0 + lane] = off_new;
    }
}

void launch_tie_patch(const TiePatchArgs& a, hipStream_t s) {
    if (a.cap) LAUNCH(tie_patch_kernel, dim3(a.cap), dim3(64), 0, s, a);
}

__global__ __launch_bounds__(64) void spec_gather_kernel(const int32_t* slots, uint32_t nlist, uint32_t ncopy, const float* s_dis,
                                                         const int64_t* s_keys, float* cdis, int64_t* ckeys) {
    const uint32_t j = blockIdx.x;
    const size_t src = (size_t)slots[j] * nlist, dst = (size_t)j * nlist;
    for (uint32_t i = threadIdx.x; i < ncopy; i += 64) {
        cdis[dst + i] = s_dis[src + i];
        ckeys[dst + i] = s_keys[src + i];
    }
}

void launch_spec_gather(const int32_t* slots, uint32_t m, uint32_t nlist, uint32_t ncopy, const float* s_dis, const int64_t* s_keys,
                        float* cdis, int64_t* ckeys, hipStream_t s) {
    if (m) LAUNCH(spec_gather_kernel, dim3(m), dim3(64), 0, s, slots, nlist, ncopy, s_dis, s_keys, cdis, ckeys);
}

__global__ __launch_bounds__(64) void gather_rows_kernel(const float* x, const uint32_t* idx, uint32_t dpad, float* out) {
    const float* src = x + (size_t)idx[blockIdx.x] * dpad;
    float* dst = out + (size_t)blockIdx.x * dpad;
    for (uint32_t i = threadIdx.x; i < dpad; i += 64) dst[i] = src[i];
}

void launch_gather_rows(const float* x, const uint32_t* idx, uint32_t m, uint32_t dpad, float* out, hipStream_t s) {
    if (m) LAUNCH(gather_rows_kernel, dim3(m), dim3(64), 0, s, x, idx, dpad, out);
}

// ... 135 lines not shown
```

### auncel_amd/csrc/ivf_select.hip

```cpp
#include "ivf_dev.h"

#include <algorithm>
#include <stdexcept>
#include <stdlib.h>
#include <string.h>
#include <string>
#include <type_traits>
#include <utility>

namespace amdivf {

struct RegHeap {
    uint32_t v0, v1;
    uint32_t s0, s1;
};

__device__ __forceinline__ void wl_u(uint32_t& reg, uint32_t val, int l) {
    uint32_t m0s;
    asm("s_mov_b32 %[m], m0\n\ts_mov_b32 m0, %[l]\n\ts_nop 0\n\tv_writelane_b32 %[r], %[v], m0\n\ts_mov_b32 m0, %[m]"
        : [r] "+v"(reg), [m] "=&s"(m0s)
        : [v] "s"(val), [l] "s"(l));
}

__device__ __forceinline__ void wl2_u(uint32_t& r0, uint32_t v0, uint32_t& r1, uint32_t v1, int l) {
// ... 42 lines not shown
    const uint32_t a = rl_u(h.p0, node & 63), b = rl_u(h.p1, node & 63);
    return node < 64 ? a : b;
}
template <bool TWO> __device__ __forceinline__ void vh_pop(VHeap& h, const VHeapLane& c, int lane, uint32_t v, uint32_t pv) {
    constexpr unsigned long long EVEN = 0x5555555555555555ull;
    const uint32_t s0 = vh_sib(h.k0), sp0 = vh_sib(h.p0);
    const unsigned long long w0 = (__ballot(h.k0 > s0) & EVEN) | (__ballot(h.k0 >= s0) & ~EVEN);
    const uint32_t t0 = vh_sel(w0, h.k0, s0), tp0 = vh_sel(w0, h.p0, sp0);
    uint32_t gk = (uint32_t)__builtin_amdgcn_ds_bpermute((int)c.caddr, (int)t0);
    uint32_t gp = (uint32_t)__builtin_amdgcn_ds_bpermute((int)c.caddr, (int)tp0);
    unsigned long long w1 = 0, path1 = 0;
    const unsigned long long low32 = 0xffffffffull;
    if (TWO) {
        const uint32_t s1 = vh_sib(h.k1), sp1 = vh_sib(h.p1);
        w1 = (__ballot(h.k1 > s1) & EVEN) | (__ballot(h.k1 >= s1) & ~EVEN);
        const uint32_t t1 = vh_sel(w1, h.k1, s1), tp1 = vh_sel(w1, h.p1, sp1);
        const uint32_t gk1 = (uint32_t)__builtin_amdgcn_ds_bpermute((int)c.caddr, (int)t1);
        const uint32_t gp1 = (uint32_t)__builtin_amdgcn_ds_bpermute((int)c.caddr, (int)tp1);
        gk = vh_sel(low32, gk, gk1);
        gp = vh_sel(low32, gp, gp1);
    } else {
        gk = vh_sel(low32, gk, 0u);
    }
    const uint32_t nlo = ~(uint32_t)w0, nhi = ~(uint32_t)(w0 >> 32);
    const unsigned long long path0 = __ballot(((nlo & c.a0lo) | (nhi & c.a0hi)) == 0u);
    if (TWO) path1 = __ballot(((nlo & c.a1lo) | (nhi & c.a1hi)) == 0u) & w1;
    const unsigned long long recv = path0 & __ballot(gk >= v);
    const unsigned long long land0 = path0 & ~recv & (__ballot(h.k0 >= v) | 2ull);
    h.k0 = vh_sel(land0, v, vh_sel(recv, gk, h.k0));
    h.p0 = vh_sel(land0, pv, vh_sel(recv, gp, h.p0));
    if (TWO) {
        const unsigned long long land1 = path1 & __ballot(h.k1 >= v);
        h.k1 = vh_sel(land1, v, h.k1);
        h.p1 = vh_sel(land1, pv, h.p1);
    }
}
template <bool TWO> __device__ __forceinline__ void vh_push(VHeap& h, const VHeapLane& c, int k, unsigned long long chain0, unsigned long long chain1,
                                                             uint32_t nv, uint32_t np) {
    const unsigned long long kbit0 = k < 64 ? 1ull << k : 0ull, kbit1 = k >= 64 ? 1ull << (k - 64) : 0ull;
    if (!(nv > vh_key_at<false>(h, k >> 1)) || k == 1) {
        h.k0 = vh_sel(kbit0, nv, h.k0);
        h.p0 = vh_sel(kbit0, np, h.p0);
        if (TWO) {
            h.k1 = vh_sel(kbit1, nv, h.k1);
            h.p1 = vh_sel(kbit1, np, h.p1);
        }
        return;
    }
    const uint32_t f0 = (uint32_t)__builtin_amdgcn_ds_bpermute((int)c.paddr0, (int)h.k0);
    const uint32_t fp0 = (uint32_t)__builtin_amdgcn_ds_bpermute((int)c.paddr0, (int)h.p0);
    const unsigned long long down0 = chain0 & ~2ull & __ballot(f0 < nv);
    const unsigned long long land0 = chain0 & (__ballot(h.k0 < nv) | kbit0) & ~down0;
    if (TWO) {
        const uint32_t f1 = (uint32_t)__builtin_amdgcn_ds_bpermute((int)c.paddr1, (int)h.k0);
        const uint32_t fp1 = (uint32_t)__builtin_amdgcn_ds_bpermute((int)c.paddr1, (int)h.p0);
        const unsigned long long down1 = chain1 & __ballot(f1 < nv);
        const unsigned long long land1 = chain1 & (__ballot(h.k1 < nv) | kbit1) & ~down1;
        h.k1 = vh_sel(land1, nv, vh_sel(down1, f1, h.k1));
        h.p1 = vh_sel(land1, np, vh_sel(down1, fp1, h.p1));
    }
    h.k0 = vh_sel(land0, nv, vh_sel(down0, f0, h.k0));
    h.p0 = vh_sel(land0, np, vh_sel(down0, fp0, h.p0));
}

__device__ __forceinline__ void rh_store(const RegHeap& h, float* hval, int64_t* href, int k, int lane, bool with_refs) {
    const bool n0 = lane >= 1 && lane <= k, n1 = lane + 64 <= k;
    int64_t r0 = 0, r1 = 0;
    if (with_refs) {
        if (n0) r0 = href[h.s0];
        if (n1) r1 = href[h.s1];
    }
    __builtin_amdgcn_fence(__ATOMIC_ACQ_REL, "wavefront");
    __builtin_amdgcn_wave_barrier();
    if (n0) hval[lane - 1] = fkey_inv(h.v0);
    if (n1) hval[lane + 63] = fkey_inv(h.v1);
    if (with_refs) {
        if (n0) href[lane - 1] = r0;
        if (n1) href[lane + 63] = r1;
    }
    __builtin_amdgcn_fence(__ATOMIC_ACQ_REL, "wavefront");
    __builtin_amdgcn_wave_barrier();
}

__device__ inline float arcos_lut(const float* lut, float x, uint32_t* err) {
    if (!(x <= 1.0 && x >= -1.0)) {
        *err = ERR_ARCOS_DOMAIN;
        return 0.f;
    }
    int index = (int)(x * 500.f / 2.f + 250.f);
    return lut[index];
}

__device__ inline float cosine_theorem_dev(float a, float b, float c, uint32_t* err) {
    if (!(a <= b)) *err = ERR_COSINE_PRECOND;
    float temp = (float)((double)a * (double)a + (double)c * (double)c - (double)b * (double)b);
    temp = temp / (2 * c);
    return c / 2 - temp;
}

__device__ inline float trace_search(const float* x, const float* z, uint32_t n, float k) {
    if (k <= x[0]) return z[0];
    if (k >= x[n - 1]) {
        const float ampli = k / x[n - 1];
        return z[n - 1] * ampli;
    }
    unsigned long long high = n - 1, low = 0, middle = 0;
    while (low <= high) {
        middle = (low + high) / 2;
        if (x[middle] < k) low = middle + 1;
        else high = middle - 1;
    }
    if (x[low] > k) low--;
    return z[low];
}

__device__ inline float kscaling_dev(float kdis, uint32_t in, const float* gt, uint32_t max_topk) {
    uint32_t index = 0;
    for (; index < max_topk; index++) {
        const float df = fabsf(gt[index] - kdis);
        if ((double)(df / kdis) < 1e-5 || (double)df < 1e-5) break;
    }
    if (index >= max_topk) return -1.f;
    return (float)(index + 1) / (float)(in + 1);
}

__device__ inline void set_online_dev(int metric, uint32_t nlist, const float* cd, const int64_t* ci,
                                      const float* interdis, const float* lut, float* dtb, int lane, uint32_t* err) {
    const uint32_t max_num = nlist / 8 + 20;
    const unsigned long long cur = (unsigned long long)ci[0];
    const float a0 = metric == METRIC_IP ? arcos_lut(lut, cd[0], err) : cd[0];
    for (uint32_t k = lane; k < max_num - 1; k += 64) {
        const unsigned long long dst = (unsigned long long)ci[k + 1];
        const unsigned long long i = cur < dst ? cur : dst, j = cur < dst ? dst : cur;
        const float c = interdis[(2ull * nlist - 1 - i) * i / 2 + j - 1 - i];
        const float b = metric == METRIC_IP ? arcos_lut(lut, cd[k + 1], err) : cd[k + 1];
        dtb[k] = cosine_theorem_dev(a0, b, c, err);
    }
    if (lane == 0) dtb[max_num - 1] = 0.f;
    if (metric == METRIC_IP) {
        for (uint32_t k = lane; k < max_num; k += 64) (void)arcos_lut(lut, cd[k], err);
    }
}

__global__ __launch_bounds__(256) void set_online_kernel(int metric, uint32_t nlist, uint32_t nq, const float* coarse_dis,
                                                         const int64_t* coarse_keys, uint32_t coarse_stride, const float* interdis,
                                                         const float* arcos, float* dtb, uint32_t* error, const uint32_t* qsel,
                                                         const uint32_t* nq_dev) {
    __shared__ float lut[500];
    for (int i = threadIdx.x; i < 500; i += 256) lut[i] = arcos[i];
    __syncthreads();
    const int lane = threadIdx.x & 63;
    const uint32_t li = blockIdx.x * 4 + (threadIdx.x >> 6);
    if (li >= (nq_dev ? *nq_dev : nq)) return;
    const uint32_t qi = qsel ? qsel[li] : li;
    uint32_t err = 0;
    set_online_dev(metric, nlist, coarse_dis + (size_t)qi * coarse_stride, coarse_keys + (size_t)qi * coarse_stride, interdis, lut,
                   dtb + (size_t)qi * (nlist / 8 + 20), lane, &err);
    err = wave_max_u32(err);
    if (err && lane == 0) atomicMax(error, err);
}

void launch_set_online(int metric, uint32_t nlist, uint32_t nq, const float* coarse_dis, const int64_t* coarse_keys,
                       uint32_t coarse_stride, const float* interdis, const float* arcos, float* dtb, uint32_t* error, hipStream_t s,
                       const uint32_t* qsel, const uint32_t* nq_dev) {
    if (nq) LAUNCH(set_online_kernel, dim3((nq + 3) / 4), dim3(256), 0, s, metric, nlist, nq, coarse_dis, coarse_keys,
                               coarse_stride, interdis, arcos, dtb, error, qsel, nq_dev);
}

__global__ __launch_bounds__(256) void partition_qsel_kernel(const uint32_t* qsel, const uint32_t* nq_dev, uint32_t nq, const int32_t* slot_of,
                                                             uint32_t* q_free, uint32_t* q_wait, uint32_t* counts) {
    const uint32_t n = nq_dev ? *nq_dev : nq;
    const int lane = threadIdx.x & 63;
    for (uint32_t i0 = (blockIdx.x * 256 + threadIdx.x) & ~63u; i0 < n; i0 += gridDim.x * 256) {
        const uint32_t i = i0 + lane;
        const bool in = i < n;
        const uint32_t q = in ? (qsel ? qsel[i] : i) : 0u;
        const bool wait = in && slot_of[q] >= 0;
        const unsigned long long mw = __ballot(wait), mf = __ballot(in && !wait);
        uint32_t bw = 0, bf = 0;
        if (lane == 0) {
            if (mw) bw = atomicAdd(&counts[1], (uint32_t)__builtin_popcountll(mw));
            if (mf) bf = atomicAdd(&counts[0], (uint32_t)__builtin_popcountll(mf));
        }
        bw = (uint32_t)__builtin_amdgcn_readfirstlane((int)bw);
        bf = (uint32_t)__builtin_amdgcn_readfirstlane((int)bf);
        const unsigned long long below = (1ull << lane) - 1ull;
        if (wait) q_wait[bw + __builtin_popcountll(mw & below)] = q;
        else if (in) q_free[bf + __builtin_popcountll(mf & below)] = q;
    }
}
void launch_partition_qsel(const uint32_t* qsel, const uint32_t* nq_dev, uint32_t nq, const int32_t* slot_of, uint32_t* q_free, uint32_t* q_wait,
                           uint32_t* counts, hipStream_t s) {
    if (!nq) return;
    const unsigned grid = std::min<unsigned>((nq + 255) / 256, 1024u);
    LAUNCH(partition_qsel_kernel, dim3(grid), dim3(256), 0, s, qsel, nq_dev, nq, slot_of, q_free, q_wait, counts);
}

__global__ __launch_bounds__(256) void small_state_kernel(SmallStateArgs a) {
    __shared__ float lut[500];
    for (int i = threadIdx.x; i < 500; i += 256) lut[i] = a.arcos[i];
    {
        const InitStateArgs& ia = a.init;
        const size_t nk = ia.n * ia.k;
        for (size_t i = threadIdx.x; i < nk; i += 256) {
            ia.heap_val[i] = ia.neutral;
            ia.heap_ref[i] = -1;
            if (ia.fix_val) {
                ia.fix_val[i] = ia.neutral;
                ia.fix_ref[i] = -1;
            }
        }
        for (size_t i = threadIdx.x; i < ia.n; i += 256) {
            ia.thr[i] = ia.neutral;
            ia.stage[i] = 0;
            ia.nscan[i] = 0;
            ia.done[i] = 0;
            ia.pre_val[i] = 0.f;
            ia.stoped[i] = 0;
            if (ia.qstat) ia.qstat[i] = make_uint2(0u, 0u);
            if (ia.log_cnt) {
                ia.log_cnt[i] = 0;
                ia.amb[i] = 0xffffffffu;
                ia.tie_flag[i] = 0;
                ia.log_snap[i] = 0;
                ia.log_snap[ia.n + i] = 0;
                ia.fin_round[i] = 0xffffffffu;
                ia.fix_pos[i] = 0;
            }
        }
        if (threadIdx.x < 4 * STATS_ROWS) ia.stats[threadIdx.x] = 0;
        if (threadIdx.x == 4 * STATS_ROWS) *ia.error = 0;
    }
    __syncthreads();
    const int lane = threadIdx.x & 63;
    const uint32_t qi = threadIdx.x >> 6;
    if (qi >= a.nq) return;
    uint32_t err = 0;
    set_online_dev(a.metric, a.nlist, a.coarse_dis + (size_t)qi * a.coarse_stride, a.coarse_keys + (size_t)qi * a.coarse_stride, a.interdis, lut,
                   a.dtb + (size_t)qi * (a.nlist / 8 + 20), lane, &err);
    err = wave_max_u32(err);
    if (err && lane == 0) atomicMax(a.init.error, err);
    if (a.ft_sorted_dis) {
        const float* od = a.ft_sorted_dis + (size_t)qi * a.ft_stride;
        uint32_t first = 0xffffffffu;
        for (uint32_t i = (uint32_t)lane; i + 1 < a.ft_nreal; i += 64)
            if (od[i] == od[i + 1] && i < first) first = i;
        for (int off = 32; off; off >>= 1) {
            const uint32_t o = (uint32_t)__shfl_xor((int)first, off);
            first = o < first ? o : first;
        }
        if (lane == 0) a.ft_out[qi] = first;
    }
    if (a.bx) {
        const int stride = (int)mfma_ksteps(a.d) * 32;
        int sq = 0, sum = 0;
        for (int c = lane * 4; c < stride; c += 256) {
            uint32_t word = 0;
#pragma unroll
            for (int b = 0; b < 4; b++) {
                int sv = 0;
                if (c + b < a.d) {
                    const int uv = (int)a.bx[(size_t)qi * a.dpad + c + b];
                    sv = uv - 128;
                    sq += sv * sv;
                    sum += uv;
                }
                word |= (uint32_t)(sv & 0xff) << (8 * b);
            }
            *reinterpret_cast<uint32_t*>(a.bout + (size_t)qi * stride + c) = word;
        }
        for (int off = 32; off; off >>= 1) {
            sq += __shfl_xor(sq, off);
            sum += __shfl_xor(sum, off);
        }
        if (lane == 0) a.bcx[qi] = a.metric == METRIC_L2 ? sq : 128 * sum - 16384 * a.d;
    }
}
void launch_small_state(const SmallStateArgs& a, hipStream_t s) { LAUNCH(small_state_kernel, dim3(1), dim3(256), 0, s, a); }
// ... 415 lines not shown
                        }
                    } else {
                        if (b0 >= n) break;
                        fetch(nv);
                    }
                    float top = RH ? unstored(rl_u(vh.k0, 1)) : hval[0];
                    uint32_t umask = 0;
#pragma unroll
                    for (int u = 0; u < NLD; u++) umask |= __ballot(hcmp<IsMax>(top, v[u])) ? (1u << u) : 0u;
                    while (umask) {
                        const int u = __builtin_ctz(umask);
                        umask &= umask - 1;
                        float x = v[0];
#pragma unroll
                        for (int t = 1; t < NLD; t++) x = t == u ? v[t] : x;
                        uint32_t cbase = b0 + u * 64;
                        if (masked) {
                            unsigned long long mm = bm;
                            for (int i = 0; i < u; i++) mm &= mm - 1;
                            cbase = (w0 - 64 + (uint32_t)__builtin_ctzll(mm)) * 64;
                        }
                        unsigned long long m = __ballot(hcmp<IsMax>(top, x));
                        while (m) {
                            const int l = __builtin_ctzll(m);
                            m &= m - 1;
                            const float val = rl_f(x, l);
                            if (hcmp<IsMax>(top, val)) {
                                const int64_t nref = refbase | (int64_t)(cbase + l);
                                if (RH) {
                                    const uint32_t sr = rl_u(vh.p0, 1);
                                    if (lane == 0) href[sr] = nref;
                                    vh_pop<VTWO>(vh, vc, lane, vh_key_at<VTWO>(vh, k), vh_pay_at<VTWO>(vh, k));
                                    vh_push<VTWO>(vh, vc, k, chain0, chain1, stored(val), sr);
                                    top = unstored(rl_u(vh.k0, 1));
                                } else {
                                    heap_pop<IsMax>(k, hval, href);
                                    heap_push<IsMax>(k, hval, href, val, nref);
                                    top = hval[0];
                                }
                                st_nheap++;
                                if (geo) {
                                    if (npend < 16) pend[npend] = val;
                                    npend++;
                                }
                            }
                        }
                    }
                    if (!masked) {
#pragma unroll
                        for (int u = 0; u < NLD; u++) v[u] = nv[u];
                        b0 += TRIP;
                    }
                }
                if (a.dbg) dbg_stream += __builtin_readcyclecounter() - dbg_s0;
                if (geo && npend) {
                    wave_sync();
                    srt_changed = true;
                    if (npend <= 16) {
                        for (uint32_t u = 0; u < npend; u++)
                            if (sorted_replace_worst<IsMax>(srt, k, pend[u], lane) < (int)query_k) top_changed = true;
                    } else {
                        if (RH) vh_store(false);
                        rank_sort_best_first<IsMax>(hval, srt, k, lane);
                        wave_sync();
                        top_changed = true;
                    }
                }
                nscan += n;
                st_ndis += n;
            }
        }
        if (a.max_codes && nscan >= a.max_codes) {
            finished = true;
            break;
        }
        if (loop_end && ik + 1 >= loop_end) finished = true;
        wave_sync();
        const unsigned long long dbg_r0 = a.dbg ? __builtin_readcyclecounter() : 0;
        if (tune) {
            const uint32_t stage = ik + 1;
            const bool overhead = a.tuner.overhead != 0;
            const bool fired = IsMax && np != 0 && !overhead;
            if (!fired) {
                uint32_t ind = 0;
                const uint32_t tmp_stage = stage >= nlist / 8 ? nlist / 8 - 1 : stage;
                while (tmp_stage > (1u << ind)) ind++;
                if ((int)ind != cached_ind) {
                    const uint32_t o = a.tuner.trace_off[ind], n = a.tuner.trace_off[ind + 1] - o;
                    const float sc = a.tuner.std_m;
                    for (uint32_t i = lane; i < n; i += 64) {
                        trc[i] = a.tuner.trace_x[o + i];
                        trc[a.trace_cap + i] = a.tuner.trace_y[o + i] + sc * a.tuner.trace_std[o + i];
                    }
                    if (lane < 15) dwin[lane] = gdtb[(1u << ind) - 1 + lane];
                    tr.n = n;
                    cached_ind = (int)ind;
                    have_pre = false;
                    wave_sync();
                }
                if (!IsMax && srt_changed) {
                    for (int i = lane; i < k; i += 64) (void)arcos_lut(lut, srt[i], &err);
                    err = wave_err(err);
                    if (err) {
                        finished = true;
                        break;
                    }
                }
                srt_changed = false;
                if (!have_pre || top_changed) {
                    dbg_evals++;
                    kept_pre = query_k <= CURNUM_PAR_MAXK ? cur_num_par<IsMax>(tr, lut, srt, dwin, terms, query_k, lane, &err)
                                                          : cur_num_lds<IsMax>(tr, lut, srt, dwin, query_k, lane, &err);
                    have_pre = true;
                    top_changed = false;
                }
                const uint32_t pre_num = kept_pre;
                float recall = (float)pre_num / (float)query_k;
                const float max_val = IsMax ? fmaxf(-1.f, srt[k - 1]) : fminf(FLT_MAX, srt[k - 1]);
                const unsigned long long stops = (unsigned long long)(racc * 12);
                if (stage > 1) {
                    if (max_val == pre_val) stoped++;
                    else stoped = 0;
                    if (stoped >= stops) recall = 1;
                }
                pre_val = max_val;
                if (!overhead) {
                    if (recall >= racc && np == 0) {
                        np = (unsigned long long)((float)stage * a.tuner.multipler);
                        if (np >= nlist && lane == 0) a.tuner.t_recalls[id_q] = 1.f;
                    }
                    if (stage >= nlist / 8 && np == 0) {
                        np = (unsigned long long)((float)stage * a.tuner.multipler);
                        if (np >= nlist && lane == 0) a.tuner.t_recalls[id_q] = 1.f;
                    }
                }
                err = wave_err(err);
                if (err) finished = true;
            }
            if (overhead) {
                if (stage >= nlist / 8) finished = true;
            } else if (np != 0 && np <= stage) {
                if (a.tuner.profile) {
                    if (RH) vh_store(false);
                    uint32_t hits = 0;
                    for (int i = lane; i < k; i += 64) {
                        const float s = hval[i];
                        if (IsMax ? ((double)s <= (double)true_KD_K * 1.0005) : ((double)s >= (double)true_KD_K * 0.9995)) hits++;
                    }
                    for (int off = 32; off; off >>= 1) hits += __shfl_xor(hits, off);
                    if (lane == 0) a.tuner.t_recalls[id_q] = (float)hits / (float)query_k;
                }
                finished = true;
            }
        }
        if (a.dbg) dbg_rule += __builtin_readcyclecounter() - dbg_r0;
        if (training && !finished) {
            const uint32_t stage = ik + 1;
            if (stage > nlist / 8) {
                finished = true;
            } else if ((stage & (stage - 1)) == 0) {
                uint32_t ind = 0;
                while (stage != (1u << ind)) ind++;
                float* out = a.train.raw[ind] + 2ull * (id_q * (unsigned long long)(k / 4));
                if (win_start != (int)(stage - 1)) {
                    wave_sync();
                    if (lane < 15) dwin[lane] = gdtb[stage - 1 + lane];
                    win_start = (int)(stage - 1);
                    wave_sync();
                }
                uint32_t count = 0;
                for (int ij = 0; ij < k; ij++) {
                    const float dv = srt[ij];
                    const float ks = kscaling_dev(dv, (uint32_t)ij, gtrow, (uint32_t)k);
                    if (ks < 0) break;
                    float tval = dv;
                    if (!IsMax) tval = arcos_lut(lut, tval, &err);
                    const float sum_a = sum_angle_par(lut, tval, dwin, lane, &err);
// ... 623 lines not shown
                            wstep = wpos >> 6;
                            W = __builtin_nontemporal_load(rmask + (size_t)wstep * 64);
                            Wn = __builtin_nontemporal_load(rmask + (size_t)(wstep + 1) * 64);
                        }
                    }
                    while (wpos < wend) {
                        const uint32_t s0 = wstep * 64u;
                        if (wpos >= s0 + 64u) {
                            W = Wn;
                            wstep++;
                            Wn = __builtin_nontemporal_load(rmask + (size_t)(wstep + 1) * 64);
                            continue;
                        }
                        const uint32_t lo = wpos - s0, hi = wend - s0 < 64u ? wend - s0 : 64u;
                        unsigned long long nz = __ballot(W != 0ull);
                        nz &= ~0ull << lo;
                        if (hi < 64u) nz &= (1ull << hi) - 1ull;
                        wpos = s0 + hi;
                        while (nz) {
                            int c0 = -1, c1 = -1, c2 = -1, c3 = -1;
                            float x0 = 0.f, x1 = 0.f, x2 = 0.f, x3 = 0.f;
                            c0 = __builtin_ctzll(nz);
                            nz &= nz - 1;
                            x0 = __builtin_nontemporal_load(region1 + (size_t)(s0 + c0) * 64);
                            if (nz) {
                                c1 = __builtin_ctzll(nz);
                                nz &= nz - 1;
                                x1 = __builtin_nontemporal_load(region1 + (size_t)(s0 + c1) * 64);
                            }
                            if (nz) {
                                c2 = __builtin_ctzll(nz);
                                nz &= nz - 1;
                                x2 = __builtin_nontemporal_load(region1 + (size_t)(s0 + c2) * 64);
                            }
                            if (nz) {
                                c3 = __builtin_ctzll(nz);
                                nz &= nz - 1;
                                x3 = __builtin_nontemporal_load(region1 + (size_t)(s0 + c3) * 64);
                            }
                            auto chunk = [&](int c, float x) {
                                if (c < 0) return;
                                if (a.dbg) dbg_chunks++;
                                const unsigned long long bits = ((unsigned long long)rl_u((uint32_t)(W >> 32), c) << 32) | rl_u((uint32_t)W, c);
                                const uint32_t cb = (s0 + (uint32_t)c - row_w0) * 64u;
                                unsigned long long m = __ballot(((bits >> lane) & 1) && hcmp<IsMax>(top, x));
                                while (m) {
                                    const int l = __builtin_ctzll(m);
                                    m &= m - 1;
                                    const float val = rl_f(x, l);
                                    const uint32_t ck = okey<IsMax>(val);
                                    if (ck < topk) admit(val, ck, lbase + cb + (uint32_t)l);
                                }
                            };
                            chunk(c0, x0);
                            chunk(c1, x1);
                            chunk(c2, x2);
                            chunk(c3, x3);
                        }
                    }
                    wpos = row_w0 + (((n + 1023u) >> 10) << 4);
                }
                nscan += n;
                st_ndis += n;
            }
        }
        flush();
        if (TUNE && st_nheap != nheap0) {
            wave_sync();
            srt_from_regs();
            wave_sync();
            srt_changed = true;
            if (ins_min < (int)query_k) top_changed = true;
        }
        if (a.max_codes && nscan >= a.max_codes) {
            finished = true;
            break;
        }
        if (loop_end && ik + 1 >= loop_end) finished = true;
        if (TUNE) {
            const unsigned long long dbg_r0 = a.dbg ? __builtin_readcyclecounter() : 0;
            const uint32_t stage = ik + 1;
            const bool fired = IsMax && np != 0 && !overhead;
            if (!fired) {
                const uint32_t tmp_stage = stage >= nl8 ? nl8 - 1 : stage;
                const uint32_t ind = tmp_stage <= 1u ? 0u : 32u - (uint32_t)__builtin_clz(tmp_stage - 1u);
                if ((int)ind != cached_ind) {
                    const uint32_t o = a.tuner.trace_off[ind], tn = a.tuner.trace_off[ind + 1] - o;
                    const float sc = a.tuner.std_m;
                    wave_sync();
                    for (uint32_t i = lane; i < tn; i += 64) {
                        trc[i] = a.tuner.trace_x[o + i];
                        trc[a.trace_cap + i] = a.tuner.trace_y[o + i] + sc * a.tuner.trace_std[o + i];
                    }
                    if (lane < 15) dwin[lane] = gdtb[(1u << ind) - 1 + lane];
                    tr.n = tn;
                    cached_ind = (int)ind;
                    have_pre = false;
                    wave_sync();
                }
                if (!IsMax && srt_changed) {
                    for (int i = lane; i < k; i += 64) (void)arcos_lut(lut, srt[i], &err);
                    err = wave_err(err);
                    if (err) {
                        finished = true;
                        break;
                    }
                }
                srt_changed = false;
                if (!have_pre || top_changed) {
                    dbg_evals++;
                    kept_pre = query_k <= CURNUM_PAR_MAXK ? cur_num_par<IsMax>(tr, lut, srt, dwin, terms, query_k, lane, &err)
                                                          : cur_num_lds<IsMax>(tr, lut, srt, dwin, query_k, lane, &err);
                    have_pre = true;
                    top_changed = false;
                    err = wave_err(err);
                    if (err) finished = true;
                    kept_recall = (float)kept_pre / (float)query_k;
                }
                float recall = kept_recall;
                const float max_val = IsMax ? fmaxf(-1.f, top) : fminf(FLT_MAX, top);
                if (stage > 1) {
                    if (max_val == pre_val) stoped++;
                    else stoped = 0;
                    if (stoped >= stops) recall = 1;
                }
                pre_val = max_val;
                if (!overhead) {
                    if (recall >= racc && np == 0) {
                        np = (unsigned long long)((float)stage * mult);
                        if (np >= nlist && lane == 0) a.tuner.t_recalls[id_q] = 1.f;
                    }
                    if (stage >= nl8 && np == 0) {
                        np = (unsigned long long)((float)stage * mult);
                        if (np >= nlist && lane == 0) a.tuner.t_recalls[id_q] = 1.f;
                    }
                }
            }
            if (overhead) {
                if (stage >= nl8) finished = true;
            } else if (np != 0 && np <= stage) {
                if (a.tuner.profile) {
                    uint32_t hits = 0;
                    for (int i = lane; i < k; i += 64) {
                        const float s = srt[i];
                        if (IsMax ? ((double)s <= (double)true_KD_K * 1.0005) : ((double)s >= (double)true_KD_K * 0.9995)) hits++;
                    }
                    for (int off = 32; off; off >>= 1) hits += __shfl_xor(hits, off);
                    if (lane == 0) a.tuner.t_recalls[id_q] = (float)hits / (float)query_k;
                }
                finished = true;
            }
            if (a.dbg) dbg_rule += __builtin_readcyclecounter() - dbg_r0;
        }
    }
    err = wave_err(err);

    if (lane == 0) {
        a.stage[qi] = ik0 + consumed;
        a.nscan[qi] = nscan;
        a.pre_val[qi] = pre_val;
        a.stoped[qi] = stoped;
        if (TUNE && np != np_in) a.tuner.my_nprobe[id_q] = np;
        if (a.qstat) {
            uint2 qs = a.qstat[qi];
            qs.x += (uint32_t)st_nlist;
            qs.y += (uint32_t)st_nheap;
            a.qstat[qi] = qs;
        }
        {
            unsigned long long* st = a.stats + 4 * xcc_id();
            if (st_nlist) xcd_local_add64(&st[0], st_nlist);
            if (st_ndis) xcd_local_add64(&st[1], st_ndis);
            if (st_nheap) xcd_local_add64(&st[2], (unsigned long long)st_nheap);
        }
        if (err) atomicMax(a.error, err);
        if (a.dbg) {
            a.dbg[(size_t)li * 8 + 0] = __builtin_readcyclecounter() - dbg_t0;
// ... 277 lines not shown
```

### include/auncel_amd.h

```cpp
#ifndef AUNCEL_AMD_H
#define AUNCEL_AMD_H
#include <stddef.h>
#include <stdint.h>

#ifdef __cplusplus
extern "C" {
#endif

#define AMD_IVF_METRIC_INNER_PRODUCT 0
#define AMD_IVF_METRIC_L2 1

typedef struct amd_ivf amd_ivf_t;

const char* amd_ivf_last_error(void);
int amd_ivf_device_count(int* count);


int amd_ivf_self_check(int device, uint64_t out[4]);

int amd_ivf_create(int d, size_t nlist, int metric, int device, amd_ivf_t** out);
int amd_ivf_destroy(amd_ivf_t* h);

int amd_ivf_clone(amd_ivf_t* h, amd_ivf_t** out);

// ... 65 lines not shown
int amd_ivf_search_exact_selected(amd_ivf_t* h, const amd_ivf_selector_t* s, size_t n, const float* x, size_t k, float* D, int64_t* I);
int amd_ivf_search_exact_resident_selected(amd_ivf_t* h, const amd_ivf_selector_t* s, size_t start, size_t n, size_t k, float* D, int64_t* I);

int amd_ivf_range_search_exact(amd_ivf_t* h, size_t n, const float* x, float radius, size_t* lims);
int amd_ivf_range_search_exact_resident(amd_ivf_t* h, size_t start, size_t n, float radius, size_t* lims);
int amd_ivf_range_search_exact_selected(amd_ivf_t* h, const amd_ivf_selector_t* s, size_t n, const float* x, float radius, size_t* lims);
int amd_ivf_last_range_exact(amd_ivf_t* h, uint64_t out[4]);

int amd_ivf_scan_codes(amd_ivf_t* h, const float* query, size_t list_no, int store_pairs, size_t k, float* simi,
                       int64_t* idxi, size_t* nup);
int amd_ivf_scan_codes_at(amd_ivf_t* h, const float* query, size_t list_no, size_t offset, size_t n, int store_pairs, size_t k,
                          float* simi, int64_t* idxi, size_t* nup);
int amd_ivf_scan_codes_range(amd_ivf_t* h, const float* query, size_t list_no, size_t offset, size_t n, float radius, size_t* count);
int amd_ivf_scan_codes_range_results(amd_ivf_t* h, uint32_t* positions, float* distances);
int amd_ivf_distance_to_code(amd_ivf_t* h, const float* query, size_t list_no, size_t offset, float* dis);

int amd_ivf_stats(amd_ivf_t* h, size_t stats[4], int reset);

int amd_ivf_coarse_resident(amd_ivf_t* h, size_t start, size_t n, size_t nprobe, float* coarse_dis, int64_t* keys, int mode);
int amd_ivf_search_resident_preassigned(amd_ivf_t* h, size_t start, size_t n, size_t k, size_t nprobe, const int64_t* keys, float* D,
                                        int64_t* I);
int amd_ivf_set_queries(amd_ivf_t* h, size_t n, const float* x);
int amd_ivf_search_resident(amd_ivf_t* h, size_t start, size_t n, size_t k, size_t nprobe, int coarse_mode, float* D,
                            int64_t* I);


int amd_ivf_set_interdis(amd_ivf_t* h, const float* table);
int amd_ivf_get_interdis(amd_ivf_t* h, float* table);

int amd_ivf_set_tuner(amd_ivf_t* h, size_t max_topk, size_t ntraces, const size_t* trace_len, const float* const* trace_x,
                      const float* const* trace_y, const float* const* trace_std, const float* arcos_list);

int amd_ivf_search_adaptive(amd_ivf_t* h, size_t start, size_t n, size_t query_topk, float multipler, float std_m,
                            const float* require_acc, const float* gt_D, int profile, int coarse_mode,
                            uint64_t* my_nprobe, float* t_recalls, float* D, int64_t* I);

int amd_ivf_search_adaptive_x(amd_ivf_t* h, size_t n, const float* x, size_t id_offset, size_t query_topk, float multipler,
                              float std_m, const float* require_acc, const float* gt_D, int profile, int coarse_mode,
                              uint64_t* my_nprobe, float* t_recalls, float* D, int64_t* I);

int amd_ivf_search_adaptive_pre(amd_ivf_t* h, size_t n, const float* x, size_t id_offset, size_t nprobe, const int64_t* keys,
                                const float* coarse_dis, size_t query_topk, float multipler, float std_m, const float* require_acc,
                                const float* gt_D, int profile, uint64_t* my_nprobe, float* t_recalls, float* D, int64_t* I);

int amd_ivf_search_timed(amd_ivf_t* h, size_t start, size_t n, size_t k, size_t nprobe, const float* budget_ms, int coarse_mode,
                         uint64_t* nprobe_used, float* D, int64_t* I);
int amd_ivf_search_timed_x(amd_ivf_t* h, size_t n, const float* x, size_t id_offset, size_t k, size_t nprobe,
                           const float* budget_ms, int coarse_mode, uint64_t* nprobe_used, float* D, int64_t* I);

int amd_ivf_train_samples(amd_ivf_t* h, size_t start, size_t n, size_t max_topk, const float* gt_D, size_t train_num,
                          int coarse_mode, float* const* raw, float* D, int64_t* I);

int amd_ivf_train_samples_x(amd_ivf_t* h, size_t n, const float* x, size_t id_offset, size_t max_topk, const float* gt_D,
                            size_t train_num, int coarse_mode, float* const* raw, float* D, int64_t* I);

int amd_ivf_train_samples_pre(amd_ivf_t* h, size_t n, const float* x, size_t id_offset, size_t nprobe, const int64_t* keys,
                              const float* coarse_dis, size_t max_topk, const float* gt_D, size_t train_num, float* const* raw,
                              float* D, int64_t* I);

int amd_ivf_arcos_table(float out[500]);

int amd_ivf_trace_sb(const float* raw_xy, size_t n, size_t bs, float* out_x, float* out_y, float* out_std,
                     size_t* nbuckets);


int amd_ivf_merge_tables(int metric, size_t n, size_t k, size_t nshard, const float* all_D, const int64_t* all_I,
                         float* D, int64_t* I);

int amd_ivf_kmeans(int d, size_t n, const float* x, size_t k, int metric, int niter, long seed, size_t max_points_per_centroid,
                   int spherical, int int_centroids, int coarse_mode, int device, float* centroids, float* obj);

int amd_ivf_range_search_preassigned(amd_ivf_t* h, size_t n, const float* x, float radius, size_t nprobe, const int64_t* keys,
                                     size_t* lims);
int amd_ivf_range_search(amd_ivf_t* h, size_t n, const float* x, float radius, size_t nprobe, int coarse_mode, size_t* lims);
int amd_ivf_range_results(amd_ivf_t* h, int64_t* labels, float* distances);


int amd_ivf_last_timing(amd_ivf_t* h, double out[8]);
int amd_ivf_last_timing_detail(amd_ivf_t* h, double out[16]);
int amd_ivf_last_scan_min_bytes(amd_ivf_t* h, double* bytes);
int amd_ivf_coarse_tie_rows(amd_ivf_t* h, uint64_t* rows);
int amd_ivf_last_tie_redone(amd_ivf_t* h, uint64_t* queries);
int amd_ivf_last_tie_patched(amd_ivf_t* h, uint64_t* rankings);
int amd_ivf_last_round_hints(amd_ivf_t* h, uint64_t out[2]);
int amd_ivf_last_tie_fixed(amd_ivf_t* h, uint64_t* queries);
int amd_ivf_last_filter(amd_ivf_t* h, uint64_t out[2]);
int amd_ivf_last_direct_out(amd_ivf_t* h);
int amd_ivf_last_coarse_pick(amd_ivf_t* h, uint64_t* rankings);

int amd_ivf_set_async_depth(amd_ivf_t* h, int depth);
int amd_ivf_submit_adaptive(amd_ivf_t* h, size_t start, size_t n, size_t query_topk, float multipler, float std_m,
                            const float* require_acc, const float* gt_D, int profile, int coarse_mode, uint64_t* my_nprobe,
                            float* t_recalls, float* D, int64_t* I, uint64_t* ticket);
int amd_ivf_submit_search_resident(amd_ivf_t* h, size_t start, size_t n, size_t k, size_t nprobe, int coarse_mode, float* D, int64_t* I,
                                   uint64_t* ticket);
int amd_ivf_submit_coarse_resident(amd_ivf_t* h, size_t start, size_t n, size_t nprobe, float* coarse_dis, int64_t* keys, int mode,
                                   uint64_t* ticket);
int amd_ivf_submit_search_resident_preassigned(amd_ivf_t* h, size_t start, size_t n, size_t k, size_t nprobe, const int64_t* keys,
                                               float* D, int64_t* I, uint64_t* ticket);
int amd_ivf_wait(amd_ivf_t* h, uint64_t ticket, double timing[9], uint64_t diag[4]);
int amd_ivf_async_counts(amd_ivf_t* h, uint64_t out[2]);

int amd_ivf_scan_arith(amd_ivf_t* h);
int amd_ivf_set_byte_codes(amd_ivf_t* h, int enable);

int amd_ivf_set_option(amd_ivf_t* h, const char* key, double value);
int amd_ivf_get_option(amd_ivf_t* h, const char* key, double* value);

int amd_ivf_read_fvecs(const char* path, size_t* d, size_t* n, float** x);
int amd_ivf_read_ivecs(const char* path, size_t* d, size_t* n, int32_t** x);
int amd_ivf_read_fbin(const char* path, size_t num, int bytes, size_t* d, size_t* n, float** x);
int amd_ivf_read_ibin(const char* path, size_t num, size_t* d, size_t* n, int32_t** x);
void amd_ivf_free(void* p);

#ifdef __cplusplus
}
#endif
#endif
```

Measured before the change: 2.974 million.

## Split tie-pending queries into tiers so most skip waiting for tie patch

```diff
diff --git a/auncel_amd/capi.py b/auncel_amd/capi.py
--- a/auncel_amd/capi.py
+++ b/auncel_amd/capi.py
@@ -25,7 +25,7 @@
     "amd_ivf_train_samples",
     "amd_ivf_train_samples_x", "amd_ivf_train_samples_pre", "amd_ivf_trace_sb", "amd_ivf_arcos_table", "amd_ivf_merge_tables",
     "amd_ivf_last_timing", "amd_ivf_last_timing_detail", "amd_ivf_last_scan_min_bytes", "amd_ivf_coarse_tie_rows", "amd_ivf_last_tie_fixed", "amd_ivf_last_filter", "amd_ivf_last_direct_out", "amd_ivf_last_coarse_pick", "amd_ivf_set_async_depth", "amd_ivf_submit_adaptive", "amd_ivf_submit_search_resident", "amd_ivf_submit_coarse_resident",
-    "amd_ivf_submit_search_resident_preassigned", "amd_ivf_wait", "amd_ivf_async_counts", "amd_ivf_last_tie_redone", "amd_ivf_last_tie_patched", "amd_ivf_self_check", "amd_ivf_last_round_hints", "amd_ivf_set_byte_codes", "amd_ivf_set_option", "amd_ivf_get_option",
+    "amd_ivf_submit_search_resident_preassigned", "amd_ivf_wait", "amd_ivf_async_counts", "amd_ivf_last_tie_redone", "amd_ivf_last_tie_patched", "amd_ivf_last_tie_tiers", "amd_ivf_self_check", "amd_ivf_last_round_hints", "amd_ivf_set_byte_codes", "amd_ivf_set_option", "amd_ivf_get_option",
     "amd_ivf_kmeans",
     "amd_ivf_range_search_preassigned", "amd_ivf_range_search", "amd_ivf_range_results",
     "amd_ivf_scan_arith",
@@ -891,6 +891,11 @@
         _chk(lib().amd_ivf_last_tie_patched(self._h, C.byref(v)))
         return int(v.value)
 
+    def last_tie_tiers(self):
+        v = (C.c_uint64 * 2)()
+        _chk(lib().amd_ivf_last_tie_tiers(self._h, v))
+        return int(v[0]), int(v[1])
+
     def last_tie_fixed(self):
         v = C.c_uint64(0)
         _chk(lib().amd_ivf_last_tie_fixed(self._h, C.byref(v)))
diff --git a/auncel_amd/csrc/ivf_dev.h b/auncel_amd/csrc/ivf_dev.h
--- a/auncel_amd/csrc/ivf_dev.h
+++ b/auncel_amd/csrc/ivf_dev.h
@@ -78,6 +78,52 @@
 __device__ __forceinline__ void wave_sync() {
     __builtin_amdgcn_fence(__ATOMIC_ACQ_REL, "wavefront");
     __builtin_amdgcn_wave_barrier();
+}
+
+__device__ inline float arcos_lut(const float* lut, float x, uint32_t* err) {
+    if (!(x <= 1.0 && x >= -1.0)) {
+        *err = ERR_ARCOS_DOMAIN;
+        return 0.f;
+    }
+    int index = (int)(x * 500.f / 2.f + 250.f);
+    return lut[index];
+}
+
+__device__ inline float cosine_theorem_dev(float a, float b, float c, uint32_t* err) {
+    if (!(a <= b)) *err = ERR_COSINE_PRECOND;
+    float temp = (float)((double)a * (double)a + (double)c * (double)c - (double)b * (double)b);
+    temp = temp / (2 * c);
+    return c / 2 - temp;
+}
+
+__device__ inline void set_online_dev(int metric, uint32_t nlist, const float* cd, const int64_t* ci,
+                                      const float* interdis, const float* lut, float* dtb, int lane, uint32_t* err) {
+    const uint32_t max_num = nlist / 8 + 20;
+    const unsigned long long cur = (unsigned long long)ci[0];
+    const float a0 = metric == METRIC_IP ? arcos_lut(lut, cd[0], err) : cd[0];
+    for (uint32_t k = lane; k < max_num - 1; k += 64) {
+        const unsigned long long dst = (unsigned long long)ci[k + 1];
+        const unsigned long long i = cur < dst ? cur : dst, j = cur < dst ? dst : cur;
+        const float c = interdis[(2ull * nlist - 1 - i) * i / 2 + j - 1 - i];
+        const float b = metric == METRIC_IP ? arcos_lut(lut, cd[k + 1], err) : cd[k + 1];
+        dtb[k] = cosine_theorem_dev(a0, b, c, err);
+    }
+    if (lane == 0) dtb[max_num - 1] = 0.f;
+    if (metric == METRIC_IP) {
+        for (uint32_t k = lane; k < max_num; k += 64) (void)arcos_lut(lut, cd[k], err);
+    }
+}
+
+constexpr uint32_t STOP_WINDOW = 15;
+__device__ __forceinline__ uint32_t stop_rule_ind(uint32_t stage, uint32_t nl8) {
+    const uint32_t tmp_stage = stage >= nl8 ? nl8 - 1 : stage;
+    return tmp_stage <= 1u ? 0u : 32u - (uint32_t)__builtin_clz(tmp_stage - 1u);
+}
+__device__ __forceinline__ uint32_t stop_window_begin(uint32_t ind) { return (1u << ind) - 1u; }
+__device__ __forceinline__ uint32_t order_read_by_first_selection(uint32_t stages, uint32_t nlist) {
+    if (stages == 0) return 0u;
+    const uint32_t window_end = stop_window_begin(stop_rule_ind(stages, nlist / 8)) + STOP_WINDOW + 1u;
+    return stages > window_end ? stages : window_end;
 }
 
 template <bool IsMax> __device__ __forceinline__ uint32_t okey(float x) {
diff --git a/auncel_amd/csrc/ivf_engine.hip b/auncel_amd/csrc/ivf_engine.hip
--- a/auncel_amd/csrc/ivf_engine.hip
+++ b/auncel_amd/csrc/ivf_engine.hip
@@ -341,10 +341,12 @@
     size_t first_tie_nreal = 0;
     DevBuf w_first_tie;
     std::vector<uint32_t> first_tie_host;
-    DevBuf w_spec_full, w_spec_dis, w_spec_keys, w_spec_count, w_spec_slot, w_spec_pick, w_redo_idx, w_spec_query, w_spec_scratch, w_split;
+    DevBuf w_spec_full, w_spec_dis, w_spec_keys, w_spec_count, w_spec_slot, w_spec_tier, w_spec_pick, w_redo_idx, w_spec_query, w_spec_scratch, w_split;
     uint32_t spec_cap = 512;
     bool spec_inline = false;
     uint32_t tie_patched_host = 0;
+    uint32_t tie_tiers_host[2] = {0, 0};
+    bool tie_tiers_valid = false;
     hipStream_t spec_stream = nullptr;
     hipEvent_t ev_spec_go = nullptr, ev_spec_done = nullptr;
     bool spec_wanted = false;
@@ -441,6 +443,7 @@
     std::vector<uint32_t> round_hint;
     uint64_t hint_sig = 0;
     uint64_t last_tie_redone = 0;
+    uint64_t last_tie_tiers[2] = {0, 0};
     uint64_t last_tie_patched = 0;
     uint32_t row_align_now = 1024;
     float* out_D = nullptr;
@@ -2521,7 +2524,7 @@
                 planned = false;
                 launch_due_fix();
                 enqueue_scan(thr_mode, nullptr, round);
-                if (round == 0 && base.split_prepare && !thr_mode && active.before == 0) {
+                if (round == 0 && base.split_prepare && !thr_mode) {
                     base.split_prepare();
                     enqueue_replay(thr_mode, (uint32_t)n, true, round, base.split_free, base.split_counts);
                     base.split_between();
@@ -3584,6 +3587,8 @@
                 d2h_small(h, h->spec_slot_host.data(), h->w_spec_slot.p, n * 4, h->stream);
                 h->tie_patched_host = 0;
                 if (h->spec_inline) d2h_small(h, &h->tie_patched_host, h->w_spec_count.as<uint32_t>() + 1, 4, h->stream);
+                h->tie_tiers_host[0] = h->tie_tiers_host[1] = 0;
+                if (h->tie_tiers_valid) d2h_small(h, h->tie_tiers_host, h->w_split.as<uint32_t>() + 1, 8, h->stream);
             }
         }
     };
@@ -3611,6 +3616,7 @@
             h->w_spec_keys.ensure((size_t)SPEC_CAP * nlist * 8);
             h->w_spec_count.ensure(32);
             h->w_spec_slot.ensure(n * 4);
+            h->w_spec_tier.ensure(n * 4);
             h->w_spec_query.ensure((size_t)SPEC_CAP * 4);
             ensure_context_streams(h);
             HIP_CHECK(hipStreamWaitEvent(h->stream, h->ev_spec_done, 0));
@@ -3618,8 +3624,8 @@
             (void)SPEC_NEAR;
             launch_tie_collect(h->w_cdis.as<float>(), (uint32_t)n, (uint32_t)h->first_tie_nreal, SPEC_WINDOW, SPEC_CAP, (uint32_t)nlist, (uint32_t)ncopy,
                                h->w_dist.as<float>(), h->w_ckeys.as<int64_t>(), h->w_first_tie.as<uint32_t>(), h->w_spec_count.as<uint32_t>(),
-                               h->w_spec_slot.as<int32_t>(), h->w_spec_full.as<float>(), h->w_spec_dis.as<float>(), h->w_spec_keys.as<int64_t>(),
-                               h->w_spec_query.as<uint32_t>(), h->stream);
+                               h->w_spec_slot.as<int32_t>(), h->w_spec_tier.as<uint32_t>(), h->w_spec_full.as<float>(), h->w_spec_dis.as<float>(),
+                               h->w_spec_keys.as<int64_t>(), h->w_spec_query.as<uint32_t>(), h->stream);
             HIP_CHECK(hipEventRecord(h->ev_spec_go, h->stream));
             HIP_CHECK(hipStreamWaitEvent(h->spec_stream, h->ev_spec_go, 0));
             launch_heap_tie_order(h->w_spec_full.as<float>(), SPEC_CAP, (uint32_t)nlist, (uint32_t)nlist, (uint32_t)ncopy, h->metric,
@@ -3659,7 +3665,7 @@
         const size_t SCRATCH_FLOATS = std::min<size_t>((size_t)64 << 20, std::max<size_t>((size_t)8 << 20, (size_t)h->spec_cap * 16 * ((maxlist + 1023) & ~(size_t)1023)));
         h->w_spec_scratch.ensure(SCRATCH_FLOATS * 4);
         base.run_ties = true;
-        base.before_first_select = [h, nlist, set_online, SCRATCH_FLOATS]() {
+        auto patch = [h, nlist, np_row, SCRATCH_FLOATS](bool tiers) {
             HIP_CHECK(hipStreamWaitEvent(h->stream, h->ev_spec_done, 0));
             TiePatchArgs ta{};
             ta.count = h->w_spec_count.as<uint32_t>();
@@ -3682,30 +3688,43 @@
             ta.scratch_floats = SCRATCH_FLOATS;
             ta.cursor = reinterpret_cast<unsigned long long*>(h->w_spec_count.as<uint32_t>() + 4);
             ta.patched = h->w_spec_count.as<uint32_t>() + 1;
+            if (tiers) {
+                ta.tier = h->w_spec_tier.as<uint32_t>();
+                ta.dtb = h->w_dtb.as<float>();
+                ta.metric = h->metric;
+                ta.cdis = h->w_cdis.as<float>();
+                ta.interdis = ix(h)->d_interdis.as<float>();
+                ta.arcos = ix(h)->d_arcos.as<float>();
+                ta.error = h->w_error.as<uint32_t>();
+            }
+            (void)np_row;
             launch_tie_patch(ta, h->stream);
+        };
+        base.before_first_select = [patch, set_online]() {
+            patch(false);
             set_online();
         };
         static const bool no_split = getenv("AUNCEL_AMD_NO_SPLIT_SELECT") != nullptr;
+        h->tie_tiers_valid = false;
         if (!no_split && n >= 256) {
             h->w_split.ensure((2 * n + 8) * 4);
             uint32_t* counts = h->w_split.as<uint32_t>();
             uint32_t* q_free = counts + 8;
             uint32_t* q_wait = q_free + n;
-            const auto patch_hook = base.before_first_select;
             const uint32_t wait_cap = (uint32_t)std::min<size_t>(n, h->spec_cap);
             base.split_free = q_free;
             base.split_wait = q_wait;
             base.split_counts = counts;
             base.split_wait_cap = wait_cap;
-            base.split_prepare = [h, n, counts, q_free, q_wait, set_online]() {
-                HIP_CHECK(hipMemsetAsync(counts, 0, 8, h->stream));
-                launch_partition_qsel(nullptr, nullptr, (uint32_t)n, h->w_spec_slot.as<int32_t>(), q_free, q_wait, counts, h->stream);
+            base.split_prepare = [h, n, nlist, counts, q_free, q_wait, set_online]() {
+                HIP_CHECK(hipMemsetAsync(counts, 0, 12, h->stream));
+                launch_partition_qsel(h->w_qsel.as<uint32_t>(), h->w_pl_counters.as<uint32_t>() + CNT_ACTIVE, (uint32_t)n, h->w_spec_slot.as<int32_t>(),
+                                      h->w_first_tie.as<uint32_t>(), h->w_pl_cnt.as<uint32_t>(), (uint32_t)nlist, h->w_spec_tier.as<uint32_t>(), q_free,
+                                      q_wait, counts, h->stream);
                 set_online();
+                h->tie_tiers_valid = true;
             };
-            base.split_between = [h, patch_hook, counts, q_wait, wait_cap, set_online]() {
-                (void)set_online;
-                patch_hook();
-            };
+            base.split_between = [patch]() { patch(true); };
         }
     }
     base.fused = ix(h)->allow_fused && ix(h)->db_range.fusable_with(qr, h->metric);
@@ -3802,6 +3821,8 @@
     }
     h->last_tie_redone = again.size();
     h->last_tie_patched = patched ? h->tie_patched_host : 0;
+    h->last_tie_tiers[0] = patched && h->tie_tiers_valid ? h->tie_tiers_host[0] : 0;
+    h->last_tie_tiers[1] = patched && h->tie_tiers_valid ? h->tie_tiers_host[1] : 0;
     if (again.empty()) return;
     const size_t m = again.size();
     std::vector<unsigned long long> nscan(n);
@@ -4326,6 +4347,12 @@
     return 0;
 }
 
+int amd_ivf_last_tie_tiers(amd_ivf_t* h, uint64_t out[2]) {
+    out[0] = h->last_tie_tiers[0];
+    out[1] = h->last_tie_tiers[1];
+    return 0;
+}
+
 int amd_ivf_last_tie_fixed(amd_ivf_t* h, uint64_t* queries) {
     API_BEGIN
     use_device(h);
diff --git a/auncel_amd/csrc/ivf_kernels.h b/auncel_amd/csrc/ivf_kernels.h
--- a/auncel_amd/csrc/ivf_kernels.h
+++ b/auncel_amd/csrc/ivf_kernels.h
@@ -341,8 +341,9 @@
 void launch_set_online(int metric, uint32_t nlist, uint32_t nq, const float* coarse_dis, const int64_t* coarse_keys,
                        uint32_t coarse_stride, const float* interdis, const float* arcos, float* dtb, uint32_t* error, hipStream_t s,
                        const uint32_t* qsel = nullptr, const uint32_t* nq_dev = nullptr);
-void launch_partition_qsel(const uint32_t* qsel, const uint32_t* nq_dev, uint32_t nq, const int32_t* slot_of, uint32_t* q_free, uint32_t* q_wait,
-                           uint32_t* counts, hipStream_t s);
+void launch_partition_qsel(const uint32_t* qsel, const uint32_t* nq_dev, uint32_t nq, const int32_t* slot_of, const uint32_t* first_tie,
+                           const uint32_t* seg_count, uint32_t nlist, uint32_t* tier, uint32_t* q_free, uint32_t* q_wait, uint32_t* counts,
+                           hipStream_t s);
 
 struct PlanArgs {
     uint32_t nq;
@@ -451,11 +452,18 @@
     unsigned long long scratch_floats;
     unsigned long long* cursor;
     uint32_t* patched;
+    const uint32_t* tier;
+    float* dtb;
+    int metric;
+    const float* cdis;
+    const float* interdis;
+    const float* arcos;
+    uint32_t* error;
 };
 void launch_tie_patch(const TiePatchArgs& a, hipStream_t s);
 void launch_tie_collect(const float* sorted_dis, uint32_t nq, uint32_t nreal, uint32_t window, uint32_t cap, uint32_t nlist, uint32_t ncopy,
-                        const float* full, const int64_t* ckeys, uint32_t* first_out, uint32_t* count, int32_t* slot_of, float* s_full, float* s_dis,
-                        int64_t* s_keys, uint32_t* slot_query, hipStream_t s);
+                        const float* full, const int64_t* ckeys, uint32_t* first_out, uint32_t* count, int32_t* slot_of, uint32_t* tier, float* s_full,
+                        float* s_dis, int64_t* s_keys, uint32_t* slot_query, hipStream_t s);
 void launch_spec_gather(const int32_t* slots, uint32_t m, uint32_t nlist, uint32_t ncopy, const float* s_dis, const int64_t* s_keys,
                         float* cdis, int64_t* ckeys, hipStream_t s);
 void launch_gather_rows(const float* x, const uint32_t* idx, uint32_t m, uint32_t dpad, float* out, hipStream_t s);
diff --git a/auncel_amd/csrc/ivf_kernels.hip b/auncel_amd/csrc/ivf_kernels.hip
--- a/auncel_amd/csrc/ivf_kernels.hip
+++ b/auncel_amd/csrc/ivf_kernels.hip
@@ -2162,7 +2162,8 @@
 
 __global__ __launch_bounds__(64) void tie_collect_kernel(const float* sorted_dis, uint32_t nreal, uint32_t window, uint32_t cap, uint32_t nlist,
                                                          uint32_t ncopy, const float* full, const int64_t* ckeys, uint32_t* first_out, uint32_t* count,
-                                                         int32_t* slot_of, float* s_full, float* s_dis, int64_t* s_keys, uint32_t* slot_query) {
+                                                         int32_t* slot_of, uint32_t* tier, float* s_full, float* s_dis, int64_t* s_keys,
+                                                         uint32_t* slot_query) {
     const uint32_t q = blockIdx.x, lane = threadIdx.x;
     const float* od = sorted_dis + (size_t)q * nlist;
     uint32_t first = 0xffffffffu;
@@ -2172,7 +2173,10 @@
         const uint32_t o = (uint32_t)__shfl_xor((int)first, off);
         first = o < first ? o : first;
     }
-    if (lane == 0) first_out[q] = first;
+    if (lane == 0) {
+        first_out[q] = first;
+        if (tier) tier[q] = 0;
+    }
     uint32_t slot = 0xffffffffu;
     if (lane == 0 && first < window) slot = atomicAdd(count, 1u);
     slot = (uint32_t)__builtin_amdgcn_readfirstlane((int)slot);
@@ -2194,11 +2198,11 @@
 }
 
 void launch_tie_collect(const float* sorted_dis, uint32_t nq, uint32_t nreal, uint32_t window, uint32_t cap, uint32_t nlist, uint32_t ncopy,
-                        const float* full, const int64_t* ckeys, uint32_t* first_out, uint32_t* count, int32_t* slot_of, float* s_full, float* s_dis,
-                        int64_t* s_keys, uint32_t* slot_query, hipStream_t s) {
+                        const float* full, const int64_t* ckeys, uint32_t* first_out, uint32_t* count, int32_t* slot_of, uint32_t* tier, float* s_full,
+                        float* s_dis, int64_t* s_keys, uint32_t* slot_query, hipStream_t s) {
     if (nq)
-        LAUNCH(tie_collect_kernel, dim3(nq), dim3(64), 0, s, sorted_dis, nreal, window, cap, nlist, ncopy, full, ckeys, first_out, count, slot_of, s_full,
-               s_dis, s_keys, slot_query);
+        LAUNCH(tie_collect_kernel, dim3(nq), dim3(64), 0, s, sorted_dis, nreal, window, cap, nlist, ncopy, full, ckeys, first_out, count, slot_of, tier,
+               s_full, s_dis, s_keys, slot_query);
 }
 
 void launch_first_tie(const float* sorted_dis, uint32_t nq, uint32_t stride, uint32_t nreal, uint32_t* out, hipStream_t s) {
@@ -2257,6 +2261,16 @@
     }
     if (!__ballot(changed)) return;
     if (lane == 0) atomicAdd(a.patched, 1u);
+    if (a.dtb) {
+        __threadfence();
+        wave_sync();
+        uint32_t err = 0;
+        set_online_dev(a.metric, a.nlist, a.cdis + (size_t)q * a.key_stride, a.ncopy >= a.nlist / 8 + 20 ? nk : ok, a.interdis, a.arcos,
+                       a.dtb + (size_t)q * (a.nlist / 8 + 20), (int)lane, &err);
+        err = wave_err(err);
+        if (err && lane == 0) atomicMax(a.error, err);
+    }
+    if (a.tier && a.tier[q] != 1u) return;
     if (!__ballot(in_round)) return;
     auto give_up = [&]() {
         if (lane == 0) a.slot_of[q] = -2 - (int32_t)slot;
diff --git a/auncel_amd/csrc/ivf_select.hip b/auncel_amd/csrc/ivf_select.hip
--- a/auncel_amd/csrc/ivf_select.hip
+++ b/auncel_amd/csrc/ivf_select.hip
@@ -148,21 +148,6 @@
     __builtin_amdgcn_wave_barrier();
 }
 
-__device__ inline float arcos_lut(const float* lut, float x, uint32_t* err) {
-    if (!(x <= 1.0 && x >= -1.0)) {
-        *err = ERR_ARCOS_DOMAIN;
-        return 0.f;
-    }
-    int index = (int)(x * 500.f / 2.f + 250.f);
-    return lut[index];
-}
-
-__device__ inline float cosine_theorem_dev(float a, float b, float c, uint32_t* err) {
-    if (!(a <= b)) *err = ERR_COSINE_PRECOND;
-    float temp = (float)((double)a * (double)a + (double)c * (double)c - (double)b * (double)b);
-    temp = temp / (2 * c);
-    return c / 2 - temp;
-}
 
 __device__ inline float trace_search(const float* x, const float* z, uint32_t n, float k) {
     if (k <= x[0]) return z[0];
@@ -188,24 +173,6 @@
     }
     if (index >= max_topk) return -1.f;
     return (float)(index + 1) / (float)(in + 1);
-}
-
-__device__ inline void set_online_dev(int metric, uint32_t nlist, const float* cd, const int64_t* ci,
-                                      const float* interdis, const float* lut, float* dtb, int lane, uint32_t* err) {
-    const uint32_t max_num = nlist / 8 + 20;
-    const unsigned long long cur = (unsigned long long)ci[0];
-    const float a0 = metric == METRIC_IP ? arcos_lut(lut, cd[0], err) : cd[0];
-    for (uint32_t k = lane; k < max_num - 1; k += 64) {
-        const unsigned long long dst = (unsigned long long)ci[k + 1];
-        const unsigned long long i = cur < dst ? cur : dst, j = cur < dst ? dst : cur;
-        const float c = interdis[(2ull * nlist - 1 - i) * i / 2 + j - 1 - i];
-        const float b = metric == METRIC_IP ? arcos_lut(lut, cd[k + 1], err) : cd[k + 1];
-        dtb[k] = cosine_theorem_dev(a0, b, c, err);
-    }
-    if (lane == 0) dtb[max_num - 1] = 0.f;
-    if (metric == METRIC_IP) {
-        for (uint32_t k = lane; k < max_num; k += 64) (void)arcos_lut(lut, cd[k], err);
-    }
 }
 
 __global__ __launch_bounds__(256) void set_online_kernel(int metric, uint32_t nlist, uint32_t nq, const float* coarse_dis,
@@ -234,6 +201,7 @@
 }
 
 __global__ __launch_bounds__(256) void partition_qsel_kernel(const uint32_t* qsel, const uint32_t* nq_dev, uint32_t nq, const int32_t* slot_of,
+                                                             const uint32_t* first_tie, const uint32_t* seg_count, uint32_t nlist, uint32_t* tier,
                                                              uint32_t* q_free, uint32_t* q_wait, uint32_t* counts) {
     const uint32_t n = nq_dev ? *nq_dev : nq;
     const int lane = threadIdx.x & 63;
@@ -241,12 +209,15 @@
         const uint32_t i = i0 + lane;
         const bool in = i < n;
         const uint32_t q = in ? (qsel ? qsel[i] : i) : 0u;
-        const bool wait = in && slot_of[q] >= 0;
-        const unsigned long long mw = __ballot(wait), mf = __ballot(in && !wait);
+        const bool slotted = in && slot_of[q] >= 0;
+        const bool wait = slotted && first_tie[q] < order_read_by_first_selection(seg_count[q], nlist);
+        if (slotted) tier[q] = wait ? 1u : 2u;
+        const unsigned long long mw = __ballot(wait), mf = __ballot(in && !wait), mb = __ballot(slotted && !wait);
         uint32_t bw = 0, bf = 0;
         if (lane == 0) {
             if (mw) bw = atomicAdd(&counts[1], (uint32_t)__builtin_popcountll(mw));
             if (mf) bf = atomicAdd(&counts[0], (uint32_t)__builtin_popcountll(mf));
+            if (mb) atomicAdd(&counts[2], (uint32_t)__builtin_popcountll(mb));
         }
         bw = (uint32_t)__builtin_amdgcn_readfirstlane((int)bw);
         bf = (uint32_t)__builtin_amdgcn_readfirstlane((int)bf);
@@ -255,11 +226,12 @@
         else if (in) q_free[bf + __builtin_popcountll(mf & below)] = q;
     }
 }
-void launch_partition_qsel(const uint32_t* qsel, const uint32_t* nq_dev, uint32_t nq, const int32_t* slot_of, uint32_t* q_free, uint32_t* q_wait,
-                           uint32_t* counts, hipStream_t s) {
+void launch_partition_qsel(const uint32_t* qsel, const uint32_t* nq_dev, uint32_t nq, const int32_t* slot_of, const uint32_t* first_tie,
+                           const uint32_t* seg_count, uint32_t nlist, uint32_t* tier, uint32_t* q_free, uint32_t* q_wait, uint32_t* counts,
+                           hipStream_t s) {
     if (!nq) return;
     const unsigned grid = std::min<unsigned>((nq + 255) / 256, 1024u);
-    LAUNCH(partition_qsel_kernel, dim3(grid), dim3(256), 0, s, qsel, nq_dev, nq, slot_of, q_free, q_wait, counts);
+    LAUNCH(partition_qsel_kernel, dim3(grid), dim3(256), 0, s, qsel, nq_dev, nq, slot_of, first_tie, seg_count, nlist, tier, q_free, q_wait, counts);
 }
 
 __global__ __launch_bounds__(256) void small_state_kernel(SmallStateArgs a) {
@@ -841,9 +813,7 @@
             const bool overhead = a.tuner.overhead != 0;
             const bool fired = IsMax && np != 0 && !overhead;
             if (!fired) {
-                uint32_t ind = 0;
-                const uint32_t tmp_stage = stage >= nlist / 8 ? nlist / 8 - 1 : stage;
-                while (tmp_stage > (1u << ind)) ind++;
+                const uint32_t ind = stop_rule_ind(stage, nlist / 8);
                 if ((int)ind != cached_ind) {
                     const uint32_t o = a.tuner.trace_off[ind], n = a.tuner.trace_off[ind + 1] - o;
                     const float sc = a.tuner.std_m;
@@ -851,7 +821,7 @@
                         trc[i] = a.tuner.trace_x[o + i];
                         trc[a.trace_cap + i] = a.tuner.trace_y[o + i] + sc * a.tuner.trace_std[o + i];
                     }
-                    if (lane < 15) dwin[lane] = gdtb[(1u << ind) - 1 + lane];
+                    if (lane < (int)STOP_WINDOW) dwin[lane] = gdtb[stop_window_begin(ind) + lane];
                     tr.n = n;
                     cached_ind = (int)ind;
                     have_pre = false;
@@ -1641,8 +1611,7 @@
             const uint32_t stage = ik + 1;
             const bool fired = IsMax && np != 0 && !overhead;
             if (!fired) {
-                const uint32_t tmp_stage = stage >= nl8 ? nl8 - 1 : stage;
-                const uint32_t ind = tmp_stage <= 1u ? 0u : 32u - (uint32_t)__builtin_clz(tmp_stage - 1u);
+                const uint32_t ind = stop_rule_ind(stage, nl8);
                 if ((int)ind != cached_ind) {
                     const uint32_t o = a.tuner.trace_off[ind], tn = a.tuner.trace_off[ind + 1] - o;
                     const float sc = a.tuner.std_m;
@@ -1651,7 +1620,7 @@
                         trc[i] = a.tuner.trace_x[o + i];
                         trc[a.trace_cap + i] = a.tuner.trace_y[o + i] + sc * a.tuner.trace_std[o + i];
                     }
-                    if (lane < 15) dwin[lane] = gdtb[(1u << ind) - 1 + lane];
+                    if (lane < (int)STOP_WINDOW) dwin[lane] = gdtb[stop_window_begin(ind) + lane];
                     tr.n = tn;
                     cached_ind = (int)ind;
                     have_pre = false;
diff --git a/include/auncel_amd.h b/include/auncel_amd.h
--- a/include/auncel_amd.h
+++ b/include/auncel_amd.h
@@ -171,6 +171,7 @@
 int amd_ivf_coarse_tie_rows(amd_ivf_t* h, uint64_t* rows);
 int amd_ivf_last_tie_redone(amd_ivf_t* h, uint64_t* queries);
 int amd_ivf_last_tie_patched(amd_ivf_t* h, uint64_t* rankings);
+int amd_ivf_last_tie_tiers(amd_ivf_t* h, uint64_t out[2]);
 int amd_ivf_last_round_hints(amd_ivf_t* h, uint64_t out[2]);
 int amd_ivf_last_tie_fixed(amd_ivf_t* h, uint64_t* queries);
 int amd_ivf_last_filter(amd_ivf_t* h, uint64_t out[2]);
```

Result: slower. 2.883 million (-3.0%).
